# jxbi1010/VLA-Touch

Hardware: AMD Instinct MI355X
Metric: refined action chunks/sec (RDT-1B chunk + DINOv2 x2 + pi_I) (higher is better)
Workload: dtype bf16 model, 16-bit activations in IEEE fp16 (RDT-1B --rdt-compute f16, DINOv2 tower; same width and MFMA rate as bf16)

## Files before the change

### include/vlatouch.h

```cpp
#ifndef VLATOUCH_H
#define VLATOUCH_H
#include <stddef.h>
#include <stdint.h>
#ifdef __cplusplus
extern "C" {
#endif

typedef void* vt_stream_t;
typedef struct vt_unet_s* vt_unet_t;
typedef struct vt_dino_s* vt_dino_t;
typedef struct vt_lstm_s* vt_lstm_t;
typedef struct vt_rdt_s* vt_rdt_t;
typedef struct vt_t5_s* vt_t5_t;

const char* vt_last_error(void);
int vt_version(void);
int vt_selftest_mfma(float* out_err, vt_stream_t stream);

int vt_prof_enable(int on);
int vt_prof_collect(double* total_ms, double* flops, double* bytes, long* launches);

int vt_gemm(const void* params, vt_stream_t stream);
enum { VT_ROUTE_UNSUPPORTED = 0,
       VT_ROUTE_BAD_ARG = 1,
       VT_ROUTE_REG = 2,
       VT_ROUTE_F32R = 3,
       VT_ROUTE_GLDS = 4,
       VT_ROUTE_PP = 5,
       VT_ROUTE_PT = 6,
       VT_ROUTE_PPK = 7,
       VT_ROUTE_PW = 8,
       VT_ROUTE_PWS = 9,
       VT_ROUTE_ROWSPLIT = 10 };
int vt_gemm_route_of(const void* params);
int vt_gemm_route_split(const void* params, int* head_route, int* tail_route);
int vt_pack_w32(const void* W, long ldw, void* out, int N, int K, vt_stream_t stream);
int vt_tune(int knob, int value);

int vt_attention(const void* params, vt_stream_t stream);
int vt_attention_kvt(const void* params, vt_stream_t stream);
size_t vt_attention_kvt_part_bytes(int B, int H, int Nq, int parts);
int vt_retile_kv(const void* K, const void* V, long ld, void* KV, int M, int T, int H, vt_stream_t stream);
int vt_groupnorm(const void* params, vt_stream_t stream);
int vt_rownorm(const void* x, int xdt, long ldx, void* y, int ydt, long ldy, const float* w, const float* b,
               int rows, int D, float eps, int mode, vt_stream_t stream);
int vt_action_normalize(const float* in, float* out, const float* mins, const float* maxs, long n, int dim,
                        float padding_factor, int denormalize, vt_stream_t stream);
int vt_randn(float* out, long n, void* state, int round_bf16, vt_stream_t stream);
int vt_slice_cast(const void* in, int idt, float* out, int B, int Tin, int Din, int T, int Dd, vt_stream_t stream);
int vt_cast(const void* in, int idt, long ldi, void* out, int odt, long ldo, int rows, int cols, vt_stream_t stream);

typedef struct {
  int nets;
  int input_dim;
  int input_pad;
  int cond_dim;
  int dsed;
  int n_groups;
  int ksize;
  int n_levels;
  int dims[4];
  int cdt;
  int adt;
} vt_unet_desc;
int vt_unet_create(const vt_unet_desc* desc, const void* const* weights, int n_weights, vt_unet_t* out);
void vt_unet_destroy(vt_unet_t h);
int vt_unet_num_weights(const vt_unet_desc* desc);
size_t vt_unet_workspace_bytes(vt_unet_t h, int B, int T);
int vt_unet_forward(vt_unet_t h, const float* x, const float* t_dev, float t_host, const float* cond,
                    float* out, int B, int T, void* workspace, vt_stream_t stream);
int vt_si_sample(vt_unet_t h, float* x, const float* cond, const float* noise, int n_steps, float beta_max,
                 int gamma_type, int epsilon_type, int sde_type, float* traj, int B, int T, void* workspace,
                 vt_stream_t stream);
int vt_si_sample_ex(vt_unet_t h, float* x, const float* cond, const float* noise, int n_steps, float beta_max,
                    int gamma_type, int epsilon_type, int sde_type, int backward, float score_weight, float* traj,
                    int B, int T, void* workspace, vt_stream_t stream);
size_t vt_unet_fused_bytes(vt_unet_t h);
int vt_unet_fused_pack(vt_unet_t h, void* buf, vt_stream_t stream);
int vt_unet_fused_covers(vt_unet_t h, int B, int T, int n_steps);
size_t vt_unet_fused_plan_bytes(vt_unet_t h, int B, int T, int n_steps);
int vt_headnorm(void* x, int dt, long tok_stride, int heads, long tokens, const float* w, float eps, int mode,
                vt_stream_t stream);

typedef struct {
  int hidden, layers, heads, patch, kpad;
  int cdt, adt;
  float eps;
  int no_cls;
  int act;
  int head_dim;
  int mlp_dim;
  int out_all;
  float attn_scale;
} vt_dino_desc;
int vt_dino_create(const vt_dino_desc* desc, const void* const* weights, int n_weights, vt_dino_t* out);
void vt_dino_destroy(vt_dino_t h);
int vt_dino_num_weights(const vt_dino_desc* desc);
size_t vt_dino_workspace_bytes(vt_dino_t h, int B_total, int res);
size_t vt_dino_packed_bytes(vt_dino_t h);
int vt_dino_set_packed(vt_dino_t h, void* buf, vt_stream_t stream);
int vt_dino_set_range_flag(vt_dino_t h, unsigned* word);
int vt_dino_forward(vt_dino_t h, const void* const* imgs, int ncams, int is_u8, int nhwc, float pre_scale,
                    int norm_mode, int B, int res, const float* pos_patch, float* out, float* flags_out,
                    void* workspace, vt_stream_t stream);

typedef struct {
  int vocab, d_model, heads, d_kv, d_ff, layers;
  int num_buckets, max_distance;
  float eps;
  int cdt, adt;
} vt_t5_desc;
int vt_t5_create(const vt_t5_desc* desc, const void* const* weights, int n_weights, vt_t5_t* out);
void vt_t5_destroy(vt_t5_t h);
int vt_t5_num_weights(const vt_t5_desc* desc);
size_t vt_t5_workspace_bytes(vt_t5_t h, int B, int L);
int vt_t5_forward(vt_t5_t h, const int32_t* ids, const uint8_t* mask_or_null, int B, int L, const int8_t* bucket_tab, void* out, int out_dt,
                  void* workspace, vt_stream_t stream);

int vt_mlp(const void* x, long ldx, int B, int n_layers, const int* dims ,
           const void* const* W, const float* const* b, int act, void* y, int ydt, long ldy,
           int cdt, int adt, void* tmp, vt_stream_t stream);
int vt_concat_obs(const float* cls1, const float* cls2, int dv, const float* state, int sdim, const float* forces,
                  int fdim, void* out, int odt, long ldo, int B, vt_stream_t stream);

typedef struct { int state_dim, hidden, layers, force_dim, force_pad, in_pad, cdt; } vt_lstm_desc;
int vt_lstm_create(const vt_lstm_desc* desc, const void* const* weights, int n_weights, vt_lstm_t* out);
void vt_lstm_destroy(vt_lstm_t h);
int vt_lstm_num_weights(const vt_lstm_desc* desc);
size_t vt_lstm_workspace_bytes(vt_lstm_t h, int B);
int vt_lstm_step(vt_lstm_t hd, const float* obs_cond, const float* vla_n, const float* force, float* h, float* c,
                 float* out_n, int B, void* workspace, vt_stream_t stream);
int vt_lstm_sequence(vt_lstm_t hd, const float* obs_cond, const float* vla_n, const float* force, float* h, float* c,
                     float* out_n, int B, int T, vt_stream_t stream);

typedef struct {
  int hidden, depth, heads, horizon, out_dim;
  int state_dim;
  int lang_dim, img_dim;
  int max_lang_len, img_len;
  int n_lang, n_img, n_state;
  int cdt, adt;
  int rms_mode;
} vt_rdt_desc;
int vt_rdt_create(const vt_rdt_desc* desc, const void* const* weights, int n_weights, vt_rdt_t* out);
void vt_rdt_destroy(vt_rdt_t h);
int vt_rdt_num_weights(const vt_rdt_desc* desc);
size_t vt_rdt_workspace_bytes(vt_rdt_t h, int B, int lang_len);
int vt_rdt_set_score_bounds(vt_rdt_t h, const float* bounds, int n);
int vt_rdt_set_state_precision(vt_rdt_t h, int fp32_state);
int vt_rdt_set_io_dtype(vt_rdt_t h, int io_dtype);
size_t vt_rdt_packed_bytes(vt_rdt_t h);
int vt_rdt_set_packed(vt_rdt_t h, void* buf, vt_stream_t stream);
#ifndef VT_RANGE_XN_SAT
#define VT_RANGE_XN_SAT 1u
#define VT_RANGE_NONFINITE 2u
#define VT_RANGE_GATE_SAT 4u
#define VT_RANGE_ATTN_EMPTY 8u
#endif
int vt_rdt_set_range_flag(vt_rdt_t h, unsigned* word);
int vt_rdt_forward(vt_rdt_t h, const void* x_tokens, const float* freq, const float* t_dev, float t_host, int t_is_scalar,
                   const void* lang_c, const void* img_c, const uint8_t* lang_mask, void* out, int B, int L,
                   void* workspace, vt_stream_t stream);
int vt_rdt_sample(vt_rdt_t h, const void* lang_tokens, const uint8_t* lang_mask, const void* img_tokens,
                  const void* state_tokens, const void* action_mask, const float* ctrl_freqs, const float* x_init,
                  int n_steps, const float* timesteps, const float* coef, int sample_pred, int adapted, float* out,
                  int B, int L, void* workspace, vt_stream_t stream);

size_t vt_marker_workspace_bytes(int N, int H, int W, int max_cand);
int vt_marker_detect(const uint8_t* frames, int channels, int mode, int N, int H, int W, double min_area, double max_area,
                     int max_cand, int* markers, int* counts, int max_markers, uint8_t* binary_out, void* workspace,
                     vt_stream_t stream);
int vt_marker_displacement(const int* markers, const int* counts, int N, int max_markers, const int* baseline, int n_base,
                           int* disp, double* force, vt_stream_t stream);

int vt_im2col_t(const float* x, float* out, int B, int Tin, int Tout, int Cin, int taps, int stride, int off0, vt_stream_t stream);
int vt_transpose(const float* in, float* out, int M, int N, vt_stream_t stream);
int vt_zero_stuff(const float* x, float* out, int B, int T, int C, vt_stream_t stream);
int vt_wflip(const float* W, float* WT, int Cout, int taps, int Cin, vt_stream_t stream);
int vt_colsum(const float* x, long ld, float* out, int M, int N, int accumulate, vt_stream_t stream);
int vt_add_(float* a, const float* b, long n, vt_stream_t stream);
int vt_copy_cols(const float* src, long lds, int off, float* dst, long ldd, int doff, int rows, int cols, int accumulate, vt_stream_t stream);
int vt_mish(const float* x, const float* dy, float* out, long n, vt_stream_t stream);
int vt_gn_mish_bwd(const float* c, const float* gamma, const float* beta, const float* film, const float* dout, float* dc,
                   float* dgamma_part, float* dbeta_part, float* dfilm, int B, int T, int C, int ngroups, float eps, vt_stream_t stream);
int vt_gelu(const float* x, const float* dy, float* out, long n, vt_stream_t stream);
int vt_si_qsample(const float* x0, const float* x1, const float* z, const float* t, float* xt, float* target_v, float* target_s,
                  float* target_b, float* t_clipped, int B, long per_sample, int gamma_type, float t_min, vt_stream_t stream);
int vt_si_qsample_ex(const float* x0, const float* x1, const float* z, const float* t, float* xt, float* target_v, float* target_s,
                     float* target_b, float* t_clipped, int B, long per_sample, int gamma_type, float t_min, int interpolant_type, vt_stream_t stream);
int vt_si_loss(const float* out, const float* target, float* dout, float* loss, int B, long per_sample, vt_stream_t stream);
int vt_slab_sum(const float* slabs, int S, long n, const float* bias, int N, float* out, vt_stream_t stream);
int vt_adamw(float* p, const float* g, float* m, float* v, long n, float lr, float beta1, float beta2, float eps, float weight_decay,
             int step, vt_stream_t stream);
int vt_ema_update(float* shadow, const float* p, long n, float decay, vt_stream_t stream);
int vt_train_hyper(float lr, float beta1, float beta2, int step, float ema_decay, float* out4_host);
int vt_adamw_dev(float* p, const float* g, float* m, float* v, long n, const float* hyper, float beta1, float beta2, float eps,
                 float weight_decay, vt_stream_t stream);
int vt_adamw_ema_multi(const void* table, int ntensors, long total_chunks, const float* hyper, float beta1, float beta2, float eps,
                       float weight_decay, vt_stream_t stream);
int vt_ema_update_dev(float* shadow, const float* p, long n, const float* hyper, vt_stream_t stream);
int vt_posemb(const float* t, float* out, int B, int dim, vt_stream_t stream);

int vt_lstm_cell_fwd(const float* gx, const float* gh, float* act, float* cseq, float* hseq, float* hprev, float* hcur, int B, int T, int H,
                     int t, vt_stream_t stream);
int vt_lstm_cell_bwd(const float* dhseq, const float* dh_rec, const float* act, const float* cseq, float* dc_next, float* dgates, float* dgcur,
                     int B, int T, int H, int t, vt_stream_t stream);
int vt_ln_bwd(const float* x, const float* gamma, const float* dy, float* dx, float* dyxh, int rows, int C, float eps, vt_stream_t stream);
int vt_bcast_mid(const float* src, float* dst, long ldd, int doff, int B, int T, int C, vt_stream_t stream);
int vt_sum_mid(const float* src, long lds, int off, float* out, int B, int T, int C, vt_stream_t stream);
int vt_mul_(float* a, const float* b, long n, vt_stream_t stream);
int vt_mse_residual(const float* base, const float* delta, const float* target, float* pred, float* ddelta, float* loss, long n, vt_stream_t stream);

typedef struct {
  const void *Q, *K, *V, *dO;
  void *dQ, *dK, *dV;
  float* ws;
  const unsigned char* kmask;
  long km_bs;
  long q_bs, q_rs, q_hs, k_bs, k_rs, k_hs, v_bs, v_rs, v_hs, do_bs, do_rs, do_hs;
  long dq_bs, dq_rs, dq_hs, dk_bs, dk_rs, dk_hs, dv_bs, dv_rs, dv_hs;
  int B, H, Nq, Nk, hd, dtype;
  float scale;
} VtAttnBwdParams;
int vt_attention_bwd(const VtAttnBwdParams* params, vt_stream_t stream);
long vt_attention_bwd_mfma_ws_bytes(int B, int H, int Nq, int Nk);
int vt_attention_bwd_mfma(const VtAttnBwdParams* params, void* ws2, long ws2_bytes, vt_stream_t stream);
int vt_rmsnorm_bwd(const void* x, const float* w, const void* dy, void* dx, float* dyxr, int rows, int D, float eps, int mode, int dt, vt_stream_t stream);
int vt_headnorm_bwd(const void* x, long x_stride, void* dy, long dy_stride, int heads, long tokens, const float* w, float* part, float eps,
                    int mode, int dt, vt_stream_t stream);
int vt_act_bwd(const void* x, const void* dy, void* out, long n, int act, int dt, vt_stream_t stream);
int vt_ddpm_qsample(const float* state, const float* action, const float* noise, const float* mask, const long* timesteps,
                    const float* alphas_cumprod, int num_train_timesteps, void* out, int odt, int B, int horizon, int action_dim, vt_stream_t stream);
int vt_timestep_embed(const float* t, const float* freqs, void* out, int odt, int B, int dim, vt_stream_t stream);
int vt_add_rowvec_(void* a, int dt, const float* v, long rows, long cols, vt_stream_t stream);
int vt_transpose_pad(const void* in, void* out, int dt, int M, int N, int Mp, vt_stream_t stream);
int vt_colsum_dt(const void* x, int dt, long ld, float* out, int M, int N, vt_stream_t stream);
int vt_add_dt(void* a, const void* b, long n, int dt, vt_stream_t stream);
typedef struct {
  int splits, rows_per_split, m_step;
  long ws_bytes;
} VtGemmTnPlan;
int vt_gemm_tn_plan(int M, int N, int K, VtGemmTnPlan* plan);
int vt_gemm_tn(const void* dy, long ld_dy, const void* x, long ld_x, int dt, int M, int N, int K, float* dw, float* db, void* ws, long ws_bytes, vt_stream_t stream);
int vt_copy_cols_dt(const void* src, long lds, long off, void* dst, long ldd, long doff, long rows, long cols, int dt, vt_stream_t stream);
int vt_grad_clip_multi(const void* table, int ntensors, long total_chunks, float max_norm, float* chunk_part, float* norm_coef, vt_stream_t stream);
int vt_mse_loss(const void* pred, const float* target, void* dpred, float* loss, long n, int dt, vt_stream_t stream);
int vt_mse_loss_scaled(const void* pred, const float* target, void* dpred, float* loss, long n, int dt, float grad_scale, vt_stream_t stream);
int vt_grad_unscale_clip_multi(const void* table, int ntensors, long total_chunks, float max_norm, float inv_scale, float* chunk_part, float* norm_coef,
                               int* found_inf, vt_stream_t stream);
int vt_grad_accum_multi(const void* table, const void* fresh, int ntensors, long total_chunks, float scale, int accumulate, vt_stream_t stream);
int vt_ema_multi(const void* table, int ntensors, long total_chunks, const float* hyper, vt_stream_t stream);
int vt_grad_fold_pack_multi(const void* table, const void* fresh, int ntensors, long total_chunks, float scale, int accumulate, void* comm_bf16,
                            vt_stream_t stream);
int vt_grad_unpack_multi(const void* table, const void* comm_bf16, int ntensors, long total_chunks, vt_stream_t stream);
int vt_adamw8_ema_multi(const void* table, const void* aux, const float* tables, int ntensors, long total_chunks, const float* hyper, float beta1,
                        float beta2, float eps, float weight_decay, vt_stream_t stream);
int vt_adam8_quantize(const float* x, unsigned char* codes, float* absmax, const float* tables, int signed_table, long n, vt_stream_t stream);
int vt_adam8_dequantize(const unsigned char* codes, const float* absmax, const float* tables, int signed_table, float* out, long n, vt_stream_t stream);
int vt_sample_metrics(const void* pred, int dt, const float* target, const float* mask, const float* state_norm, const int* dataset_idx, int B,
                      int H, int A, int n_datasets, float* per_sample, float* overall, double* acc, int* count, double* ws, vt_stream_t stream);

typedef struct {
  const void* src;
  const void* coef_h;
  const void* coef_v;
  long pitch;
  int h, w;
  int out_h, out_w;
  int ksize_h, ksize_v;
  int rows_max;
  int reserved;
  long out_off;
  long ws_off;
} vt_imgprep_frame;
#define VT_IMGPREP_PAD 1
#define VT_IMGPREP_BRIGHT 2
#define VT_IMGPREP_OUT_BF16 4
#define VT_IMGPREP_OUT_U8 8
#define VT_IMGPREP_TWO_PASS 16
size_t vt_imgprep_workspace_bytes(vt_imgprep_frame* frames_host, int n, int S, int flags);
int vt_imgprep(const vt_imgprep_frame* frames_host, const void* frames_dev, int n, int S, const void* lut, unsigned fill_rgb, int flags,
               void* out, void* ws, size_t ws_bytes, vt_stream_t stream);

typedef struct {
  const void* src;
  long pitch;
  int h, w;
  long out_off;
  int order[4];
  float brightness, contrast, saturation;
  unsigned char hue_shift;
  unsigned char reserved[3];
} vt_colorjitter_frame;
#define VT_COLORJITTER_BRIGHTNESS 0
#define VT_COLORJITTER_CONTRAST 1
#define VT_COLORJITTER_SATURATION 2
#define VT_COLORJITTER_HUE 3
#define VT_COLORJITTER_NONE 4
#define VT_COLORJITTER_LIFT 1
size_t vt_colorjitter_workspace_bytes(int n);
int vt_colorjitter(const vt_colorjitter_frame* frames_host, const void* frames_dev, int n, int flags, void* out, void* ws, size_t ws_bytes,
                   vt_stream_t stream);

typedef struct {
  const void* src;
  long pitch;
  int h, w;
  long out_off;
  long ws_off;
} vt_jpegmap_frame;
#define VT_JPEGMAP_CV2_ORDER 1
size_t vt_jpegmap_workspace_bytes(vt_jpegmap_frame* frames_host, int n);
int vt_jpegmap(const vt_jpegmap_frame* frames_host, const void* frames_dev, int n, int quality, int flags, void* out, void* ws,
               size_t ws_bytes, vt_stream_t stream);

#define VT_RDT_MASK_FREQ 1
#define VT_RDT_MASK_STATE 2
#define VT_RDT_MASK_ELEM 4
#define VT_RDT_NOISE 8
int vt_rdt_batch(const double* qpos, const int* ep_off, const double* ep_stats, const double* ds_mean, const int* col_map, const float* lang,
                 const int* lang_off, int E, int S, int A, int H, int D, int Lmax, int ctrl_freq, double noise_div, const void* plan, int B,
                 float* states, float* actions, float* elem_mask, float* state_norm, long long* ctrl_freqs, float* lang_out,
                 unsigned char* lang_mask, vt_stream_t stream);

#define VT_CTRL_BRIDGE 0
#define VT_CTRL_LSTM 1
int vt_ctrl_batch(const double* pose10, const double* vla, const float* forces, const int* ep_off, const float* feat, const unsigned long long* pix_sum,
                  int E, long long rows, int Hv, int Fd, int dv, long long P, const float* stats, float padding_factor, int cf, int h, int layout,
                  int use_force, const int* plan, int B, float* obs_in, int in_pad, float* expert_act, float* vla_act, float* forces_out,
                  float* current_force, float* norm_flags, vt_stream_t stream);
int vt_ctrl_pixsum(const unsigned char* frames, long long P, int n, unsigned long long* sums, vt_stream_t stream);

#ifdef __cplusplus
}
#endif
#endif
```

### vla-touch_amd/csrc/vt_api.hip

```cpp
#include <string.h>
#include "vt_common.h"
#include "vt_kernels.h"
#include "vt_host.h"
#include "vt_gemm_route.h"
#include "vt_prof.h"
#include "vt_unet_int.h"
#include "../../include/vlatouch.h"

VtProfState g_vt_prof;

extern "C" {

const char* vt_last_error(void) { return vt_errbuf(); }
int vt_version(void) { return 100; }

int vt_gemm(const void* params, vt_stream_t stream) {
  if (!params) return vt_fail(VT_ERR_ARG, "vt_gemm: null params");
  const int r = vt_gemm_launch(*reinterpret_cast<const VtGemmParams*>(params), (hipStream_t)stream);
  if (r) vt_fail(r, "vt_gemm: rejected (alignment: K, lda, ldw multiples of 8 bf16 / 4 fp32; conv: cin likewise) or launch failure");
  return r;
}
int vt_gemm_route_of(const void* params) {
  if (!params) return VT_ROUTE_BAD_ARG;
  return vt_gemm_route(*reinterpret_cast<const VtGemmParams*>(params));
}
int vt_gemm_route_split(const void* params, int* head_route, int* tail_route) {
  if (!params || !head_route || !tail_route) return vt_fail(VT_ERR_ARG, "vt_gemm_route_split: null argument");
  const VtGemmParams& p = *reinterpret_cast<const VtGemmParams*>(params);
  if (vt_gemm_route(p) != VT_GEMM_ROWSPLIT) return vt_fail(VT_ERR_ARG, "vt_gemm_route_split: the block does not route to VT_ROUTE_ROWSPLIT");
  VtGemmParams head, tail;
  *head_route = vt_gemm_rowsplit(p, head, tail);
  *tail_route = vt_gemm_route(tail);
  return VT_OK;
}
int vt_tune(int knob, int value) {
  if (knob == 1 && (value == 0 || value == 4 || value == 8)) { vt_gemm_pw_tune(value); return VT_OK; }
  if (knob == 2 || knob == 8) { vt_gemm_route_tune(knob, value); return VT_OK; }
  if (knob == 4) { vt_gemm_pws_tune(value); return VT_OK; }
  if (knob == 6) { vt_attn_kvt_tune(value); return VT_OK; }
  if (knob == 7) { vt_unet_fused_tune(value); return VT_OK; }
  if (knob == 9 && (value == 0 || value == 1 || value == 3 || value == 6)) { vt_attn16g_tune(value); return VT_OK; }
  return vt_fail(VT_ERR_ARG, "vt_tune: unknown knob %d / value %d", knob, value);
}
int vt_prof_enable(int on) {
  g_vt_prof.on = on != 0;
  g_vt_prof.mode = on > 1 ? on : 1;
  if (on) { g_vt_prof.used = 0; g_vt_prof.flops = 0.0; g_vt_prof.bytes = 0.0; }
  return VT_OK;
}
int vt_prof_collect(double* total_ms, double* flops, double* bytes, long* launches) {
  double ms = 0.0;
  for (int i = 0; i < g_vt_prof.used; ++i) {
    float t = 0.f;
    if (hipEventElapsedTime(&t, g_vt_prof.ev[2 * i], g_vt_prof.ev[2 * i + 1]) != hipSuccess) return VT_ERR_LAUNCH;
    ms += t;
  }
  if (total_ms) *total_ms = ms;
  if (flops) *flops = g_vt_prof.flops;
  if (bytes) *bytes = g_vt_prof.bytes;
  if (launches) *launches = g_vt_prof.used;
  return VT_OK;
}
int vt_attention(const void* params, vt_stream_t stream) {
  if (!params) return vt_fail(VT_ERR_ARG, "vt_attention: null params");
  const int r = vt_attn_launch(*reinterpret_cast<const VtAttnParams*>(params), (hipStream_t)stream);
  if (r) vt_fail(r, "vt_attention: bad strides/sizes or launch failure");
  return r;
}
int vt_attention_kvt(const void* params, vt_stream_t stream) {
  if (!params) return vt_fail(VT_ERR_ARG, "vt_attention_kvt: null params");
  const int r = vt_attn_kvt_launch(*reinterpret_cast<const VtAttnKvtParams*>(params), (hipStream_t)stream);
  if (r) vt_fail(r, "vt_attention_kvt: bad sizes / strides (T * 64 >= B * Nk, q_rs % 8), parts without part_ws or > 16, or launch failure");
  return r;
}
size_t vt_attention_kvt_part_bytes(int B, int H, int Nq, int parts) { return vt_attn_kvt_part_bytes(B, H, Nq, parts); }
int vt_retile_kv(const void* K, const void* V, long ld, void* KV, int M, int T, int H, vt_stream_t stream) {
  if (!K || !V || !KV || M < 1 || H < 1) return vt_fail(VT_ERR_ARG, "vt_retile_kv: null source / destination or empty shape");
  const int r = vt_k_retile_kv(K, V, ld, KV, M, T, H, (hipStream_t)stream);
  if (r) vt_fail(r, "vt_retile_kv: T * 64 < M, ld % 8 or launch failure");
  return r;
}
int vt_groupnorm(const void* params, vt_stream_t stream) {
  if (!params) return vt_fail(VT_ERR_ARG, "vt_groupnorm: null params");
  const int r = vt_k_groupnorm(*reinterpret_cast<const VtGnParams*>(params), (hipStream_t)stream);
  if (r) vt_fail(r, "vt_groupnorm: unsupported group size or launch failure");
  return r;
}
int vt_rownorm(const void* x, int xdt, long ldx, void* y, int ydt, long ldy, const float* w, const float* b, int rows, int D, float eps,
               int mode, vt_stream_t stream) {
  const int r = vt_k_rownorm(x, xdt, ldx, y, ydt, ldy, w, b, rows, D, eps, mode, (hipStream_t)stream);
  if (r) vt_fail(r, "vt_rownorm: D must be a multiple of 4 and <= 2048");
  return r;
}
int vt_headnorm(void* x, int dt, long tok_stride, int heads, long tokens, const float* w, float eps, int mode, vt_stream_t stream) {
  return vt_k_headnorm(x, dt, tok_stride, heads, tokens, w, eps, mode, (hipStream_t)stream);
}
int vt_action_normalize(const float* in, float* out, const float* mins, const float* maxs, long n, int dim, float padding_factor,
                        int denormalize, vt_stream_t stream) {
  if (!in || !out || !mins || !maxs || n < 0 || dim < 1) return vt_fail(VT_ERR_ARG, "vt_action_normalize: bad argument");
  if (n == 0) return VT_OK;
  return vt_k_actnorm(in, out, mins, maxs, n, dim, padding_factor, denormalize, (hipStream_t)stream);
}

}

static_assert(VT_ROUTE_UNSUPPORTED == VT_GEMM_UNSUPPORTED && VT_ROUTE_BAD_ARG == VT_GEMM_BAD_ARG && VT_ROUTE_REG == VT_GEMM_REG && VT_ROUTE_F32R == VT_GEMM_F32R &&
              VT_ROUTE_GLDS == VT_GEMM_GLDS && VT_ROUTE_PP == VT_GEMM_PP && VT_ROUTE_PT == VT_GEMM_PT && VT_ROUTE_PPK == VT_GEMM_PPK && VT_ROUTE_PW == VT_GEMM_PW &&
              VT_ROUTE_PWS == VT_GEMM_PWS && VT_ROUTE_ROWSPLIT == VT_GEMM_ROWSPLIT, "include/vlatouch.h route codes = enum VtGemmRoute");

namespace {
template <typename T>
__global__ void mfma_selftest_kernel(float* err) {
  const int lane = threadIdx.x, g = lane >> 4, l15 = lane & 15;
  Frag<T> a, b;
  float av[8], bv[8];
  for (int j = 0; j < 8; ++j) {
    const int k = g * 8 + j;
    av[j] = (k == l15) ? 1.f : 0.f;
    bv[j] = (float)(l15 * 100 + k);
  }
  if constexpr (sizeof(T) == 2) {
    for (int j = 0; j < 8; ++j) { a.v[j] = (short)f2bf(av[j]); b.v[j] = (short)f2bf(bv[j]); }
  } else {
    for (int j = 0; j < 8; ++j) { a.v[j] = av[j]; b.v[j] = bv[j]; }
  }
  float4_t acc = {0.f, 0.f, 0.f, 0.f};
  mma16(acc, a, b);
  float e = 0.f;
  for (int r = 0; r < 4; ++r) {
    const int row = g * 4 + r, col = l15;
    float expect = (float)(col * 100 + row);
    if constexpr (sizeof(T) == 2) expect = bf2f(f2bf(expect));
    e = fmaxf(e, fabsf(acc[r] - expect));
  }
  e = wave_max(e);
  if (lane == 0) *err = e;
}
}

extern "C" int vt_selftest_mfma(float* out_err, vt_stream_t stream) {
  if (!out_err) return vt_fail(VT_ERR_ARG, "vt_selftest_mfma: null");
  hipLaunchKernelGGL((mfma_selftest_kernel<bf16_t>), dim3(1), dim3(64), 0, (hipStream_t)stream, out_err);
  hipLaunchKernelGGL((mfma_selftest_kernel<float>), dim3(1), dim3(64), 0, (hipStream_t)stream, out_err + 1);
  return vt_check_launch();
}

namespace {
__device__ __forceinline__ void philox_round(uint32_t (&c)[4], const uint32_t k0, const uint32_t k1) {
  const uint64_t p0 = (uint64_t)0xD2511F53u * c[0], p1 = (uint64_t)0xCD9E8D57u * c[2];
  const uint32_t n0 = (uint32_t)(p1 >> 32) ^ c[1] ^ k0, n1 = (uint32_t)p1, n2 = (uint32_t)(p0 >> 32) ^ c[3] ^ k1, n3 = (uint32_t)p0;
  c[0] = n0; c[1] = n1; c[2] = n2; c[3] = n3;
}
__device__ __forceinline__ void philox4x32_10(uint32_t (&c)[4], uint32_t k0, uint32_t k1) {
#pragma unroll
  for (int r = 0; r < 10; ++r) { philox_round(c, k0, k1); k0 += 0x9E3779B9u; k1 += 0xBB67AE85u; }
}
__global__ void randn_kernel(float* __restrict__ out, const long n, const unsigned long long* __restrict__ state, const int round_bf16) {
  const long q = (long)blockIdx.x * blockDim.x + threadIdx.x;
  if (q * 4 >= n) return;
  const unsigned long long key = state[0], ctr = state[1] + (unsigned long long)q;
  uint32_t c[4] = {(uint32_t)ctr, (uint32_t)(ctr >> 32), 0u, 0u};
  philox4x32_10(c, (uint32_t)key, (uint32_t)(key >> 32));
  float v[4];
#pragma unroll
  for (int h = 0; h < 2; ++h) {
    const float u1 = ((float)(c[2 * h] >> 8) + 0.5f) * (1.0f / 16777216.0f);
    const float u2 = ((float)(c[2 * h + 1] >> 8) + 0.5f) * (1.0f / 16777216.0f);
    const float r = sqrtf(-2.0f * __logf(u1));
    float sn, cs;
    __sincosf(6.283185307179586f * u2, &sn, &cs);
    v[2 * h] = r * cs; v[2 * h + 1] = r * sn;
  }
#pragma unroll
  for (int j = 0; j < 4; ++j) {
    if (round_bf16) v[j] = bf2f(f2bf(v[j]));
    if (q * 4 + j < n) out[q * 4 + j] = v[j];
  }
}
__global__ void randn_advance_kernel(unsigned long long* state, const unsigned long long by) { state[1] += by; }
template <typename TI>
__global__ void slice_cast_kernel(const TI* __restrict__ in, float* __restrict__ out, int B, int Tin, int Din, int T, int Dd) {
  const long i = (long)blockIdx.x * blockDim.x + threadIdx.x;
  if (i >= (long)B * T * Dd) return;
  const int d = (int)(i % Dd);
  const long r = i / Dd;
  const int t = (int)(r % T), b = (int)(r / T);
  out[i] = Elem<TI>::to_f(in[((long)b * Tin + t) * Din + d]);
}
}

extern "C" int vt_randn(float* out, long n, void* state, int round_bf16, vt_stream_t stream) {
  if (!out || !state || n < 0) return vt_fail(VT_ERR_ARG, "vt_randn: null argument");
  if (n == 0) return VT_OK;
  const long quads = (n + 3) / 4;
  hipLaunchKernelGGL(randn_kernel, dim3((unsigned)((quads + 255) / 256)), dim3(256), 0, (hipStream_t)stream, out, n, (const unsigned long long*)state, round_bf16);
  hipLaunchKernelGGL(randn_advance_kernel, dim3(1), dim3(1), 0, (hipStream_t)stream, (unsigned long long*)state, (unsigned long long)quads);
  return vt_check_launch();
}
extern "C" int vt_slice_cast(const void* in, int idt, float* out, int B, int Tin, int Din, int T, int Dd, vt_stream_t stream) {
  if (!in || !out || B < 1 || T < 1 || Dd < 1 || T > Tin || Dd > Din) return vt_fail(VT_ERR_ARG, "vt_slice_cast: bad shape");
  const long n = (long)B * T * Dd;
  const dim3 grid((unsigned)((n + 255) / 256));
  if (idt == VT_BF16) hipLaunchKernelGGL((slice_cast_kernel<bf16_t>), grid, dim3(256), 0, (hipStream_t)stream, (const bf16_t*)in, out, B, Tin, Din, T, Dd);
  else if (idt == VT_F32) hipLaunchKernelGGL((slice_cast_kernel<float>), grid, dim3(256), 0, (hipStream_t)stream, (const float*)in, out, B, Tin, Din, T, Dd);
  else return vt_fail(VT_ERR_UNSUPPORTED, "vt_slice_cast: bf16 or fp32 input");
  return vt_check_launch();
}

extern "C" int vt_cast(const void* in, int idt, long ldi, void* out, int odt, long ldo, int rows, int cols, vt_stream_t stream) {
  if (!in || !out || rows < 1 || cols < 1) return vt_fail(VT_ERR_ARG, "vt_cast: bad argument");
  const int r = vt_k_act_copy(in, idt, ldi, out, odt, ldo, rows, cols, VT_ACT_NONE, (hipStream_t)stream);
  if (r) vt_fail(r, "vt_cast: unsupported dtype pair");
  return r;
}
```

### vla-touch_amd/csrc/vt_common.h

```cpp
#pragma once
#include <hip/hip_runtime.h>
#include <stdint.h>
#include <type_traits>

typedef uint16_t bf16_t;
typedef __attribute__((ext_vector_type(8))) short short8_t;
typedef __attribute__((ext_vector_type(4))) float float4_t;
typedef __attribute__((ext_vector_type(8))) __bf16 bf16x8_t;
typedef __attribute__((ext_vector_type(8))) _Float16 f16x8_t;
struct half_t { uint16_t b; };
typedef __attribute__((ext_vector_type(4))) short short4_t;
typedef __attribute__((ext_vector_type(4))) int int4_t;
typedef __attribute__((ext_vector_type(16))) float float16_t;
typedef __attribute__((address_space(3))) void lds_void;
typedef const __attribute__((address_space(1))) void glb_void;
typedef __attribute__((address_space(3))) short4_t lds_short4_t;

#define VT_OK 0
#define VT_ERR_ARG (-22)
#define VT_ERR_LAUNCH (-5)
#define VT_ERR_UNSUPPORTED (-95)

enum { VT_F32 = 0, VT_BF16 = 1, VT_F32X3 = 2, VT_F16 = 3 };
enum { VT_ACT_NONE = 0, VT_ACT_GELU_ERF = 1, VT_ACT_GELU_TANH = 2, VT_ACT_SILU = 3, VT_ACT_MISH = 4,
       VT_ACT_SWIGLU = 5,
       VT_ACT_GEGLU = 6 };

__device__ __forceinline__ float bf2f(bf16_t h) { return __uint_as_float(((uint32_t)h) << 16); }
typedef __attribute__((ext_vector_type(2))) float float2_t;
typedef __attribute__((ext_vector_type(2))) __bf16 bf16x2_t;
__device__ __forceinline__ uint32_t pk_bf16(float lo, float hi) {
  return __builtin_bit_cast(uint32_t, __builtin_convertvector((float2_t){lo, hi}, bf16x2_t));
}
typedef __attribute__((ext_vector_type(2))) _Float16 f16x2_t;
template <typename T> __device__ __forceinline__ uint32_t pk16(float lo, float hi);
template <> __device__ __forceinline__ uint32_t pk16<bf16_t>(float lo, float hi) { return pk_bf16(lo, hi); }
template <> __device__ __forceinline__ uint32_t pk16<half_t>(float lo, float hi) {
  return __builtin_bit_cast(uint32_t, __builtin_convertvector((float2_t){lo, hi}, f16x2_t));
}
template <typename T> __host__ __device__ constexpr short one16() { return std::is_same<T, half_t>::value ? (short)0x3C00 : (short)0x3F80; }
__device__ __forceinline__ bf16_t f2bf(float f) { return __builtin_bit_cast(bf16_t, (__bf16)f); }
__device__ __forceinline__ float h2f(half_t h) { return (float)__builtin_bit_cast(_Float16, h.b); }
__device__ __forceinline__ half_t f2h(float f) { half_t r; r.b = __builtin_bit_cast(uint16_t, (_Float16)f); return r; }

template <typename T> struct Elem;
template <> struct Elem<float> {
  static constexpr int EPC = 4;
  __device__ static __forceinline__ float to_f(float v) { return v; }
  __device__ static __forceinline__ float from_f(float v) { return v; }
};
template <> struct Elem<bf16_t> {
  static constexpr int EPC = 8;
  __device__ static __forceinline__ float to_f(bf16_t v) { return bf2f(v); }
  __device__ static __forceinline__ bf16_t from_f(float v) { return f2bf(v); }
};
template <> struct Elem<half_t> {
  static constexpr int EPC = 8;
  __device__ static __forceinline__ float to_f(half_t v) { return h2f(v); }
  __device__ static __forceinline__ half_t from_f(float v) { return f2h(v); }
};

template <typename T> struct Frag;
template <> struct Frag<bf16_t> { short8_t v; };
template <> struct Frag<half_t> { short8_t v; };
template <> struct Frag<float> { float v[8]; };

__device__ __forceinline__ void mma16(float4_t& acc, const Frag<bf16_t>& a, const Frag<bf16_t>& b) {
  acc = __builtin_amdgcn_mfma_f32_16x16x32_bf16(__builtin_bit_cast(bf16x8_t, a.v), __builtin_bit_cast(bf16x8_t, b.v), acc, 0, 0, 0);
}
__device__ __forceinline__ void mma16(float4_t& acc, const Frag<half_t>& a, const Frag<half_t>& b) {
  acc = __builtin_amdgcn_mfma_f32_16x16x32_f16(__builtin_bit_cast(f16x8_t, a.v), __builtin_bit_cast(f16x8_t, b.v), acc, 0, 0, 0);
}
__device__ __forceinline__ void mma16(float4_t& acc, const Frag<float>& a, const Frag<float>& b) {
#pragma unroll
  for (int j = 0; j < 8; ++j) acc = __builtin_amdgcn_mfma_f32_16x16x4f32(a.v[j], b.v[j], acc, 0, 0, 0);
}

template <typename T16> __device__ __forceinline__ float16_t mma32(const int4_t w, const int4_t a, const float16_t c);
template <> __device__ __forceinline__ float16_t mma32<bf16_t>(const int4_t w, const int4_t a, const float16_t c) {
  return __builtin_amdgcn_mfma_f32_32x32x16_bf16(__builtin_bit_cast(bf16x8_t, w), __builtin_bit_cast(bf16x8_t, a), c, 0, 0, 0);
}
template <> __device__ __forceinline__ float16_t mma32<half_t>(const int4_t w, const int4_t a, const float16_t c) {
  return __builtin_amdgcn_mfma_f32_32x32x16_f16(__builtin_bit_cast(f16x8_t, w), __builtin_bit_cast(f16x8_t, a), c, 0, 0, 0);
}

template <int N, typename F> __device__ __forceinline__ void static_for(F&& f) {
  if constexpr (N > 0) { static_for<N - 1>(f); f(std::integral_constant<int, N - 1>{}); }
}

#ifdef VLATOUCH_DRAIN_WAITS
#define VT_VMCNT(N) 0
#else
#define VT_VMCNT(N) N
#endif
template <int N> __device__ __forceinline__ void vt_wait_vm() { asm volatile("s_waitcnt vmcnt(%0)" ::"n"(VT_VMCNT(N)) : "memory"); }
template <int N> __device__ __forceinline__ void vt_wait_vm(int4_t (&w)[4]) {
  asm volatile("s_waitcnt vmcnt(%[n])" : "+v"(w[0]), "+v"(w[1]), "+v"(w[2]), "+v"(w[3]) : [n] "i"(VT_VMCNT(N)) : "memory");
}
template <int N> __device__ __forceinline__ void vt_wait_vm(int4_t (&w)[8]) {
  asm volatile("s_waitcnt vmcnt(%[n])" : "+v"(w[0]), "+v"(w[1]), "+v"(w[2]), "+v"(w[3]), "+v"(w[4]), "+v"(w[5]), "+v"(w[6]), "+v"(w[7]) : [n] "i"(VT_VMCNT(N)) : "memory");
}

template <int OFF, bool FIRST>
__device__ __forceinline__ void wload(int4_t& d, const unsigned voff, const char* sbase) {
  if constexpr (FIRST) asm volatile("s_nop 4\n\tglobal_load_dwordx4 %0, %1, %2 offset:%3" : "=v"(d) : "v"(voff), "s"(sbase), "i"(OFF) : "memory");
  else asm volatile("global_load_dwordx4 %0, %1, %2 offset:%3" : "=v"(d) : "v"(voff), "s"(sbase), "i"(OFF) : "memory");
}
#define VT_UNIFORM_PTR(p)                                                                                                             \
  reinterpret_cast<const char*>(((unsigned long)(unsigned)__builtin_amdgcn_readfirstlane((int)((unsigned long)(p) >> 32)) << 32) | \
                                (unsigned long)(unsigned)__builtin_amdgcn_readfirstlane((int)(unsigned long)(p)))

__device__ __forceinline__ int swz(int row, int chunk) { return chunk ^ ((row >> 1) & 7); }

__device__ __forceinline__ void lds_frag(Frag<bf16_t>& f, const char* tile, int row, int k8) {
  f.v = *reinterpret_cast<const short8_t*>(tile + row * 128 + swz(row, k8) * 16);
}
__device__ __forceinline__ void lds_frag(Frag<half_t>& f, const char* tile, int row, int k8) {
  f.v = *reinterpret_cast<const short8_t*>(tile + row * 128 + swz(row, k8) * 16);
}
__device__ __forceinline__ void lds_frag(Frag<float>& f, const char* tile, int row, int k8) {
  const float4_t lo = *reinterpret_cast<const float4_t*>(tile + row * 128 + swz(row, 2 * k8) * 16);
  const float4_t hi = *reinterpret_cast<const float4_t*>(tile + row * 128 + swz(row, 2 * k8 + 1) * 16);
  f.v[0] = lo[0]; f.v[1] = lo[1]; f.v[2] = lo[2]; f.v[3] = lo[3];
  f.v[4] = hi[0]; f.v[5] = hi[1]; f.v[6] = hi[2]; f.v[7] = hi[3];
}

template <typename T>
__device__ __forceinline__ void tr_frag_half(Frag<T>& f, const int hh, const char* a) {
  const short4_t t = __builtin_amdgcn_ds_read_tr16_b64_v4i16((lds_short4_t*)a);
  f.v[hh * 4 + 0] = t[0]; f.v[hh * 4 + 1] = t[1]; f.v[hh * 4 + 2] = t[2]; f.v[hh * 4 + 3] = t[3];
}

__device__ __forceinline__ float fast_exp(float x) { return __builtin_amdgcn_exp2f(x * 1.4426950408889634f); }

__device__ __forceinline__ float fast_erf(float x) {
  const float ax = fabsf(x);
  const float t = __builtin_amdgcn_rcpf(1.0f + 0.3275911f * ax);
  const float p = t * (0.254829592f + t * (-0.284496736f + t * (1.421413741f + t * (-1.453152027f + t * 1.061405429f))));
  return copysignf(1.0f - p * fast_exp(-ax * ax), x);
}

__device__ __forceinline__ float act_apply(float x, int act) {
  switch (act) {
    case VT_ACT_GELU_ERF: return 0.5f * x * (1.0f + fast_erf(x * 0.70710678118654752440f));
    case VT_ACT_GELU_TANH: {
      const float u2 = 1.5957691216057308f * (x + 0.044715f * x * x * x);
      return x * __builtin_amdgcn_rcpf(1.0f + fast_exp(-u2));
    }
    case VT_ACT_SILU: return x * __builtin_amdgcn_rcpf(1.0f + fast_exp(-x));
    case VT_ACT_MISH: {
      if (x > 20.0f) return x;
      const float n = fast_exp(x), w = n * (n + 2.0f);
      return x * w * __builtin_amdgcn_rcpf(w + 2.0f);
    }
    default: return x;
  }
}

template <int W, bool MAX> __device__ __forceinline__ float rows_pair(float v) {
  static_assert(W == 16 || W == 32, "a row is 16 lanes: pairs of rows, then pairs of pairs");
  const unsigned u = __builtin_bit_cast(unsigned, v);
  float a0, a1;
  if constexpr (W == 16) {
    const auto a = __builtin_amdgcn_permlane16_swap(u, u, false, false);
    a0 = __builtin_bit_cast(float, (unsigned)a[0]); a1 = __builtin_bit_cast(float, (unsigned)a[1]);
  } else {
    const auto a = __builtin_amdgcn_permlane32_swap(u, u, false, false);
    a0 = __builtin_bit_cast(float, (unsigned)a[0]); a1 = __builtin_bit_cast(float, (unsigned)a[1]);
  }
  return MAX ? fmaxf(a0, a1) : a0 + a1;
}
__device__ __forceinline__ float rows4_sum(float v) { return rows_pair<32, false>(rows_pair<16, false>(v)); }
__device__ __forceinline__ float rows4_max(float v) { return rows_pair<32, true>(rows_pair<16, true>(v)); }
__device__ __forceinline__ float row16_sum(float v) {
  auto dpp = [](float x, auto ctrl) {
    return __int_as_float(__builtin_amdgcn_update_dpp(0, __float_as_int(x), decltype(ctrl)::value, 0xf, 0xf, false));
  };
  v += dpp(v, std::integral_constant<int, 0xB1>{});
  v += dpp(v, std::integral_constant<int, 0x4E>{});
  v += dpp(v, std::integral_constant<int, 0x141>{});
  v += dpp(v, std::integral_constant<int, 0x140>{});
  return v;
}
__device__ __forceinline__ float row16_max(float v) {
  auto dpp = [](float x, auto ctrl) {
    return __int_as_float(__builtin_amdgcn_update_dpp(0, __float_as_int(x), decltype(ctrl)::value, 0xf, 0xf, false));
  };
  v = fmaxf(v, dpp(v, std::integral_constant<int, 0xB1>{}));
  v = fmaxf(v, dpp(v, std::integral_constant<int, 0x4E>{}));
  v = fmaxf(v, dpp(v, std::integral_constant<int, 0x141>{}));
  v = fmaxf(v, dpp(v, std::integral_constant<int, 0x140>{}));
  return v;
}
__device__ __forceinline__ float wave_sum(float v) { return rows4_sum(row16_sum(v)); }
__device__ __forceinline__ float wave_max(float v) { return rows4_max(row16_max(v)); }

template <typename T> __device__ __forceinline__ float ldf(const T* p, size_t i);
template <> __device__ __forceinline__ float ldf<float>(const float* p, size_t i) { return p[i]; }
template <> __device__ __forceinline__ float ldf<bf16_t>(const bf16_t* p, size_t i) { return bf2f(p[i]); }
template <> __device__ __forceinline__ float ldf<half_t>(const half_t* p, size_t i) { return h2f(p[i]); }
template <typename T> __device__ __forceinline__ void stf(T* p, size_t i, float v);
template <> __device__ __forceinline__ void stf<float>(float* p, size_t i, float v) { p[i] = v; }
template <> __device__ __forceinline__ void stf<bf16_t>(bf16_t* p, size_t i, float v) { p[i] = f2bf(v); }
template <> __device__ __forceinline__ void stf<half_t>(half_t* p, size_t i, float v) { p[i] = f2h(v); }

__device__ __forceinline__ float vt_actnorm(float x, float mn, float mx, float pad, int denorm) {
  const float pr = (mx - mn) * pad;
  const float ctr = (mn + mx) / 2;
  const float pmin = ctr - pr / 2, pmax = ctr + pr / 2;
  float rng = pmax - pmin;
  if (denorm) return (x + 1.0f) / 2.0f * rng + pmin;
  if (rng < 1e-6f) rng = 1.0f;
  return 2.0f * (x - pmin) / rng - 1.0f;
}

#ifndef VT_RANGE_XN_SAT
#define VT_RANGE_XN_SAT 1u
#define VT_RANGE_NONFINITE 2u
#define VT_RANGE_GATE_SAT 4u
#define VT_RANGE_ATTN_EMPTY 8u
#endif
__device__ __forceinline__ void vt_range_note(unsigned* flag, unsigned bit) {
  if (flag) __hip_atomic_fetch_or(flag, bit, __ATOMIC_RELAXED, __HIP_MEMORY_SCOPE_AGENT);
}
__device__ __forceinline__ bool vt_nonfinite(float v) { return !(fabsf(v) <= 3.4028234664e38f); }

static inline int vt_check_launch() { return hipGetLastError() == hipSuccess ? VT_OK : VT_ERR_LAUNCH; }

#define DISPATCH_T(dt, T, ...) \
  if ((dt) == VT_F32) { using T = float; __VA_ARGS__; } else if ((dt) == VT_F16) { using T = half_t; __VA_ARGS__; } else { using T = bf16_t; __VA_ARGS__; }
#define DISPATCH_T16(dt, T, ...) \
  if ((dt) == VT_F16) { using T = half_t; __VA_ARGS__; } else { using T = bf16_t; __VA_ARGS__; }
static inline bool vt_is_act_dtype(int dt) { return dt == VT_F32 || dt == VT_BF16 || dt == VT_F16; }
```

### vla-touch_amd/csrc/vt_gemm_pw.hip

```cpp
#include "vt_common.h"
#include "vt_gemm_route.h"
#include "vt_gemm_epilogue.h"
#include "vt_prof.h"
#include "vt_host.h"
#include "vt_kernels.h"
#include "../../include/vlatouch.h"

namespace {

constexpr int BM = 160, BN = 128, BK = 64;
constexpr int TMW = BM / 32;
constexpr int A_TILE = BM * 128;
constexpr int OPS = BM / 8 / 4 + 4;

template <typename T16, typename TC, int NB, int FUSE = 0>
__global__ __launch_bounds__(256, 1) void gemm_pw_kernel(const VtGemmParams p, const int tiles_n, const int tiles_per_group, const int total_tiles, const int GM) {
  constexpr int SMEM = NB * A_TILE > BM * BN * 4 ? NB * A_TILE : BM * BN * 4;
  __shared__ __attribute__((aligned(16))) char smem[SMEM];
  const int tid = threadIdx.x, lane = tid & 63;
  const int wave = __builtin_amdgcn_readfirstlane(tid >> 6);
  const int l31 = lane & 31, hk = lane >> 5;

  int bid = blockIdx.x;
  if ((total_tiles & 7) == 0) bid = (bid & 7) * (total_tiles >> 3) + (bid >> 3);
  const int grp = bid / tiles_per_group;
  const int t_in = bid - grp * tiles_per_group;
  const int tiles_m = tiles_per_group / tiles_n;
  const int sr = t_in / (GM * tiles_n);
  const int gmr = min(GM, tiles_m - sr * GM);
  const int r_in = t_in - sr * GM * tiles_n;
  const int tn = r_in / gmr, tm = sr * GM + (r_in - tn * gmr);
  const int m0 = tm * BM, n0 = tn * BN;

  const uint16_t* A = reinterpret_cast<const uint16_t*>(p.A) + (long)grp * p.a_gs;
  const int nk = p.K / BK;

  const __amdgpu_buffer_rsrc_t rsA = __builtin_amdgcn_make_buffer_rsrc((void*)(A + (long)m0 * p.lda), 0, 0x7fffffff, 0x00020000);
  int asrc[5];
#pragma unroll
  for (int e = 0; e < 5; ++e) {
    const int r = (wave + 4 * e) * 8 + (lane >> 3);
    const int c = (lane & 7) ^ ((r >> 1) & 7);
    asrc[e] = (int)(((long)(min(m0 + r, p.M - 1) - m0) * p.lda + c * 8) * 2);
  }
  const char* wbase = reinterpret_cast<const char*>(p.Wp) + ((long)grp * p.w_gs) * 2 + ((long)(n0 / 32 + wave) * (p.K / 16)) * 1024;
  wbase = VT_UNIFORM_PTR(wbase);
  const unsigned wvoff = lane * 16;

  int4_t wb[NB][4];
  auto issue = [&](const int kt, auto bc) {
    constexpr int b = decltype(bc)::value;
#pragma unroll
    for (int e = 0; e < 5; ++e)
      __builtin_amdgcn_raw_ptr_buffer_load_lds(rsA, (lds_void*)(smem + b * A_TILE + (wave + 4 * e) * 1024), 16, asrc[e], kt * (BK * 2), 0, 0);
    const char* sb = wbase + (long)kt * 4096;
    wload<0, true>(wb[b][0], wvoff, sb);
    wload<1024, false>(wb[b][1], wvoff, sb);
    wload<2048, false>(wb[b][2], wvoff, sb);
    wload<3072, false>(wb[b][3], wvoff, sb);
  };

  const int xr = (l31 >> 1) & 7;
  int foff[4];
#pragma unroll
  for (int s = 0; s < 4; ++s) foff[s] = l31 * 128 + (((s * 2 + hk) ^ xr) * 16);
  auto frags = [&](int4_t (&f)[TMW], const int b, const int s) {
#pragma unroll
    for (int j = 0; j < TMW; ++j) f[j] = *reinterpret_cast<const int4_t*>(smem + b * A_TILE + j * 4096 + foff[s]);
  };

  float16_t acc[TMW];
#pragma unroll
  for (int j = 0; j < TMW; ++j)
#pragma unroll
    for (int r = 0; r < 16; ++r) acc[j][r] = 0.f;

  static_for<NB - 1>([&](auto bc) { if (decltype(bc)::value < nk) issue(decltype(bc)::value, bc); });
  vt_wait_vm<(NB - 3) * OPS>(wb[0]);
  vt_wait_vm<(NB - 3) * OPS>(wb[1]);
  __builtin_amdgcn_sched_barrier(0);
  __builtin_amdgcn_s_barrier();
  __builtin_amdgcn_sched_barrier(0);
  int4_t af[2][TMW];
  frags(af[0], 0, 0);

  constexpr int RSV = FUSE == 2 ? (BM * 16 + 255) / 256 : 1;
  float4 rsv[RSV];
  auto sub = [&](const int t, auto uc, auto tailc) {
    constexpr int U = decltype(uc)::value;
    constexpr bool TAIL = decltype(tailc)::value;
    if constexpr (!TAIL || U == 0) issue(t + NB - 1, std::integral_constant<int, (U + NB - 1) % NB>{});
    if constexpr (FUSE == 2 && TAIL && U == NB - 2) {
      const int h2 = p.rs_n >> 1, nq = BM * h2;
#pragma unroll
      for (int i = 0; i < RSV; ++i) {
        const int q = tid + 256 * i;
        const int row = q / h2, c = q - row * h2;
        rsv[i] = q < nq ? *reinterpret_cast<const float4*>(p.rs_part + ((long)min(m0 + row, p.M - 1) * p.rs_n + 2 * c) * 2) : make_float4(0.f, 0.f, 0.f, 0.f);
      }
    }
#pragma unroll
    for (int s = 0; s < 4; ++s) {
      if (s < 3) frags(af[(s + 1) & 1], U, s + 1);
      else if (!TAIL || U < NB - 1) frags(af[0], (U + 1) % NB, 0);
#pragma unroll
      for (int j = 0; j < TMW; ++j) acc[j] = mma32<T16>(wb[U][s], af[s & 1][j], acc[j]);
    }
#pragma unroll
    for (int i = 0; i < 4 * TMW; ++i) {
      __builtin_amdgcn_sched_group_barrier(0x008, 1, 0);
      __builtin_amdgcn_sched_group_barrier(0x100, 1, 0);
    }
    if constexpr (!TAIL) vt_wait_vm<(NB - 3) * OPS>(wb[(U + 2) % NB]);
    else if constexpr (U + 2 < NB) vt_wait_vm<(NB - 3 - U > 0 ? NB - 3 - U : 0) * OPS>(wb[(U + 2) % NB]);
    __builtin_amdgcn_sched_barrier(0);
    __builtin_amdgcn_s_barrier();
    __builtin_amdgcn_sched_barrier(0);
  };
  int t = 0;
  for (; t + NB < nk; t += NB) static_for<NB>([&](auto uc) { sub(t + decltype(uc)::value, uc, std::false_type{}); });
  static_for<NB>([&](auto uc) { sub(t + decltype(uc)::value, uc, std::true_type{}); });

  float* tile = reinterpret_cast<float*>(smem);
  float rs[TMW];
#pragma unroll
  for (int j = 0; j < TMW; ++j) rs[j] = 1.f;
  if constexpr (FUSE == 2) {
    float2* pair = reinterpret_cast<float2*>(tile + BM);
    const int h2 = p.rs_n >> 1;
#pragma unroll
    for (int i = 0; i < RSV; ++i) {
      const int q = tid + 256 * i;
      if (q < BM * h2) {
        const float dS = rsv[i].y - rsv[i].w;
        pair[q] = make_float2(rsv[i].x + rsv[i].z + (p.rs_mode == 2 ? dS * dS * (1.0f / 128.0f) : 0.f), rsv[i].y + rsv[i].w);
      }
    }
    __syncthreads();
    if (tid < BM) {
      float var;
      if (p.rs_mode == 2) {
        float na = 0.f, mean = 0.f, m2 = 0.f;
        for (int c = 0; c < h2; ++c) {
          const float2 v = pair[tid * h2 + c];
          const float delta = v.y * (1.0f / 128.0f) - mean, nt = na + 128.0f;
          mean += delta * (128.0f / nt);
          m2 += v.x + delta * delta * (na * 128.0f / nt);
          na = nt;
        }
        var = m2 / (1.0f / p.rs_inv_k - 1.0f);
      } else {
        float sq = 0.f;
        for (int c = 0; c < h2; ++c) sq += pair[tid * h2 + c].x;
        var = sq * p.rs_inv_k;
      }
      tile[tid] = rsqrtf(var + p.rs_eps);
    }
    __syncthreads();
#pragma unroll
    for (int j = 0; j < TMW; ++j) rs[j] = tile[j * 32 + l31];
    __syncthreads();
  }
  const int half = wave & 1, c4 = lane & 15;
  const int ncol0 = n0 + half * 64, n = ncol0 + c4 * 4;
  const bool col_ok = n < p.N;
  const int rbase = (wave >> 1) * (BM / 2) + (lane >> 4);
  TC* Cg = reinterpret_cast<TC*>(p.C) + (long)grp * p.c_gs;
  const TC* Rg = p.residual ? reinterpret_cast<const TC*>(p.residual) + (long)grp * p.r_gs : nullptr;
  constexpr bool PRE = sizeof(TC) == 4;
  float4 rpre[PRE ? BM / 8 : 1];
  const bool use_pre = PRE && Rg != nullptr;
  if constexpr (PRE) {
    if (use_pre) {
#pragma unroll
      for (int it = 0; it < BM / 8; ++it) {
        const int m = min(m0 + rbase + it * 4, p.M - 1);
        rpre[it] = col_ok ? *reinterpret_cast<const float4*>(reinterpret_cast<const float*>(Rg) + (long)m * p.ldr + n) : make_float4(0.f, 0.f, 0.f, 0.f);
      }
    }
  }
  const float* bias = p.bias ? p.bias + (long)grp * p.bias_gs : nullptr;
  const float* hw = nullptr;
  if (p.hn_w0 && ncol0 < p.hn_c0_end) hw = p.hn_w0;
  else if (p.hn_w1 && ncol0 >= p.hn_c0_end && ncol0 < p.hn_c1_end) hw = p.hn_w1;
  const float4 zero4 = make_float4(0.f, 0.f, 0.f, 0.f), one4 = make_float4(1.f, 1.f, 1.f, 1.f);
  const float4 b4 = (bias && col_ok) ? *reinterpret_cast<const float4*>(bias + n) : zero4;
  const float4 cs4 = (p.colscale && col_ok) ? *reinterpret_cast<const float4*>(p.colscale + n) : one4;
  const float4 hw4 = hw ? *reinterpret_cast<const float4*>(hw + c4 * 4) : one4;
  float4 g4 = zero4;
  if constexpr (FUSE == 1) { if (col_ok && p.xn_gain) g4 = *reinterpret_cast<const float4*>(p.xn_gain + n); }
  __builtin_amdgcn_sched_barrier(0);
  constexpr int PFN = 8;
  unsigned pfv[PFN];
#pragma unroll
  for (int i = 0; i < PFN; ++i) pfv[i] = 0;
  if (p.pf_ptr) {
    const unsigned nbytes = (unsigned)p.pf_bytes;
    const unsigned share = ((nbytes + (unsigned)total_tiles - 1u) / (unsigned)total_tiles + 63u) & ~63u;
    const unsigned b0 = blockIdx.x * share;
    const __amdgpu_buffer_rsrc_t rsP = __builtin_amdgcn_make_buffer_rsrc((void*)((const char*)p.pf_ptr + b0), 0,
                                                                        b0 < nbytes ? (int)min(share, nbytes - b0) : 0, 0x00020000);
#pragma unroll
    for (int i = 0; i < PFN; ++i)
      if ((unsigned)i * 16384u < share) pfv[i] = __builtin_amdgcn_raw_buffer_load_b32(rsP, (i * 256 + tid) * 64, 0, 0);
  }
  __builtin_amdgcn_sched_barrier(0);
#pragma unroll
  for (int j = 0; j < TMW; ++j) {
    const int m = j * 32 + l31;
    const float r = FUSE == 2 ? rs[j] : 1.f;
#pragma unroll
    for (int rq = 0; rq < 4; ++rq) {
      const int n4 = wave * 8 + rq * 2 + hk;
      *reinterpret_cast<float4*>(tile + m * BN + ((n4 ^ (m & 7)) * 4)) =
          make_float4(acc[j][rq * 4] * r, acc[j][rq * 4 + 1] * r, acc[j][rq * 4 + 2] * r, acc[j][rq * 4 + 3] * r);
    }
  }
  __syncthreads();
  if (p.act != VT_ACT_NONE) {
#pragma unroll 2
    for (int it = 0; it < BM / 8; ++it) {
      const int row = rbase + it * 4;
      const float4 x = *reinterpret_cast<const float4*>(tile + row * BN + (((half * 16 + c4) ^ (row & 7)) * 4));
      vt_epi_segment<TC, 0, true>(p, x, b4, cs4, hw, hw4, Cg, Rg, m0 + row, n, ncol0, col_ok);
    }
  } else if (FUSE == 1 && PRE && use_pre) {
    if constexpr (PRE && FUSE == 1) {
      T16* Xn = reinterpret_cast<T16*>(p.xn_out);
      const int pcol = 2 * tn + half, pn = 2 * tiles_n;
#pragma unroll
      for (int it = 0; it < BM / 8; ++it) {
        const int row = rbase + it * 4, m = m0 + row;
        const float4 x = *reinterpret_cast<const float4*>(tile + row * BN + (((half * 16 + c4) ^ (row & 7)) * 4));
        float o[4] = {x.x + b4.x, x.y + b4.y, x.z + b4.z, x.w + b4.w};
        o[0] *= cs4.x; o[1] *= cs4.y; o[2] *= cs4.z; o[3] *= cs4.w;
        o[0] += rpre[it].x; o[1] += rpre[it].y; o[2] += rpre[it].z; o[3] += rpre[it].w;
        const bool ok = m < p.M && col_ok;
        const float q1 = row16_sum(ok ? (o[0] + o[1]) + (o[2] + o[3]) : 0.f);
        float q;
        if (p.rs_mode == 2) {
          const float mj = q1 * (1.0f / 64.0f);
          const float d0 = o[0] - mj, d1 = o[1] - mj, d2 = o[2] - mj, d3 = o[3] - mj;
          q = row16_sum(ok ? (d0 * d0 + d1 * d1) + (d2 * d2 + d3 * d3) : 0.f);
        } else q = row16_sum(ok ? (o[0] * o[0] + o[1] * o[1]) + (o[2] * o[2] + o[3] * o[3]) : 0.f);
        if (ok) {
          vt_epi_st128(reinterpret_cast<float*>(Cg) + (long)m * p.ldc + n, make_float4(o[0], o[1], o[2], o[3]));
          constexpr float LIM = std::is_same<T16, half_t>::value ? 65504.0f : 3.0e38f;
          auto sat = [](float v) { return fminf(fmaxf(v, -LIM), LIM); };
          const float xg[4] = {o[0] * g4.x, o[1] * g4.y, o[2] * g4.z, o[3] * g4.w};
          if constexpr (std::is_same<T16, half_t>::value) {
            if (fmaxf(fmaxf(fabsf(xg[0]), fabsf(xg[1])), fmaxf(fabsf(xg[2]), fabsf(xg[3]))) > LIM) vt_range_note(p.range_flag, VT_RANGE_XN_SAT);
          }
          T16 ov[4] = {Elem<T16>::from_f(sat(xg[0])), Elem<T16>::from_f(sat(xg[1])), Elem<T16>::from_f(sat(xg[2])), Elem<T16>::from_f(sat(xg[3]))};
          vt_epi_st64(Xn + (long)m * p.xn_ld + n, *reinterpret_cast<const uint2*>(ov));
        }
        if (c4 == 0 && m < p.M) *reinterpret_cast<float2*>(p.xn_part + ((long)m * pn + pcol) * 2) = make_float2(q, q1);
      }
    }
  } else if (use_pre) {
#pragma unroll
    for (int it = 0; it < BM / 8; ++it) {
      const int row = rbase + it * 4;
      const float4 x = *reinterpret_cast<const float4*>(tile + row * BN + (((half * 16 + c4) ^ (row & 7)) * 4));
      vt_epi_segment<TC, 0, false>(p, x, b4, cs4, hw, hw4, Cg, nullptr, m0 + row, n, ncol0, col_ok, &rpre[PRE ? it : 0]);
    }
  } else {
#pragma unroll 4
    for (int it = 0; it < BM / 8; ++it) {
      const int row = rbase + it * 4;
      const float4 x = *reinterpret_cast<const float4*>(tile + row * BN + (((half * 16 + c4) ^ (row & 7)) * 4));
      vt_epi_segment<TC, 0, false>(p, x, b4, cs4, hw, hw4, Cg, Rg, m0 + row, n, ncol0, col_ok);
    }
  }
#pragma unroll
  for (int i = 0; i < PFN; ++i) asm volatile("" :: "v"(pfv[i]));
}

__global__ void pack_w32_kernel(const uint16_t* __restrict__ W, const long ldw, uint16_t* __restrict__ out, const int N, const int K) {
  const long i = (long)blockIdx.x * blockDim.x + threadIdx.x;
  const long nchunks = (long)N * K / 8;
  if (i >= nchunks) return;
  const int lane = (int)(i & 63);
  const long frag = i >> 6;
  const int ks = (int)(frag % (K / 16));
  const int nt = (int)(frag / (K / 16));
  const int n = nt * 32 + (lane & 31), k = ks * 16 + (lane >> 5) * 8;
  *reinterpret_cast<uint4*>(out + i * 8) = *reinterpret_cast<const uint4*>(W + (long)n * ldw + k);
}

}

static int g_vt_pw_nb = 0;

void vt_gemm_pw_tune(int ring) { g_vt_pw_nb = ring; }

bool vt_gemm_pw_fits(const VtGemmParams& p) {
  if (!p.Wp || p.cmap || p.groups != 1) return false;
  if (p.N % BN || p.K % (8 * BK) || p.lda >= (1 << 21)) return false;
  const long tiles = (long)((p.M + BM - 1) / BM) * (p.N / BN) * p.groups;
  const long rounds = (tiles + 255) / 256;
  return tiles >= 100 && tiles * 8 >= rounds * 256 * 7;
}

int vt_gemm_pw_launch(const VtGemmParams& p, hipStream_t s) {
  const int tiles_n = p.N / BN, tiles_m = (p.M + BM - 1) / BM;
  const int per_group = tiles_n * tiles_m, total = per_group * p.groups;
  const int gm = 4;
  VtProfScope prof(3, p, s);
  const bool c16 = p.c_dtype != VT_F32;
#define VT_PW_GO(T16, TC) do { if (g_vt_pw_nb == 8) hipLaunchKernelGGL((gemm_pw_kernel<T16, TC, 8>), dim3(total), dim3(256), 0, s, p, tiles_n, per_group, total, gm); \
                               else hipLaunchKernelGGL((gemm_pw_kernel<T16, TC, 4>), dim3(total), dim3(256), 0, s, p, tiles_n, per_group, total, gm); } while (0)
  if (p.xn_out || p.rs_part) {
    const dim3 g(total), b(256);
    if (p.xn_out && (c16 || !p.residual || p.act != VT_ACT_NONE || p.hn_w0 || p.hn_w1)) return VT_ERR_UNSUPPORTED;
    if (p.xn_out && p.rs_part) return VT_ERR_UNSUPPORTED;
    if (p.xn_out) {
      if (p.a_dtype == VT_BF16) hipLaunchKernelGGL((gemm_pw_kernel<bf16_t, float, 4, 1>), g, b, 0, s, p, tiles_n, per_group, total, gm);
      else hipLaunchKernelGGL((gemm_pw_kernel<half_t, float, 4, 1>), g, b, 0, s, p, tiles_n, per_group, total, gm);
    } else if (!c16) {
      return VT_ERR_UNSUPPORTED;
    } else if (p.a_dtype == VT_BF16) {
      hipLaunchKernelGGL((gemm_pw_kernel<bf16_t, bf16_t, 4, 2>), g, b, 0, s, p, tiles_n, per_group, total, gm);
    } else {
      hipLaunchKernelGGL((gemm_pw_kernel<half_t, half_t, 4, 2>), g, b, 0, s, p, tiles_n, per_group, total, gm);
    }
    return vt_check_launch();
  }
  if (p.a_dtype == VT_BF16) { if (c16) VT_PW_GO(bf16_t, bf16_t); else VT_PW_GO(bf16_t, float); }
  else { if (c16) VT_PW_GO(half_t, half_t); else VT_PW_GO(half_t, float); }
#undef VT_PW_GO
  return vt_check_launch();
}

extern "C" int vt_pack_w32(const void* W, long ldw, void* out, int N, int K, vt_stream_t stream) {
  if (!W || !out || N <= 0 || K <= 0 || N % 32 || K % 16 || ldw % 8) return vt_fail(VT_ERR_ARG, "vt_pack_w32: N %% 32, K %% 16, ldw %% 8 must be 0");
  const long nchunks = (long)N * K / 8;
  hipLaunchKernelGGL(pack_w32_kernel, dim3((unsigned)((nchunks + 255) / 256)), dim3(256), 0, (hipStream_t)stream, (const uint16_t*)W, ldw, (uint16_t*)out, N, K);
  return vt_check_launch();
}
```

### vla-touch_amd/csrc/vt_gemm_route.h

```cpp
#pragma once
#include <hip/hip_runtime.h>
#include "vt_gemm.h"

enum VtGemmRoute : int {
  VT_GEMM_UNSUPPORTED = 0,
  VT_GEMM_BAD_ARG = 1,
  VT_GEMM_REG = 2,
  VT_GEMM_F32R = 3,
  VT_GEMM_GLDS = 4,
  VT_GEMM_PP = 5,
  VT_GEMM_PT = 6,
  VT_GEMM_PPK = 7,
  VT_GEMM_PW = 8,
  VT_GEMM_PWS = 9,
  VT_GEMM_ROWSPLIT = 10,
};

VtGemmRoute vt_gemm_route(const VtGemmParams& p);
VtGemmRoute vt_gemm_rowsplit(const VtGemmParams& p, VtGemmParams& head, VtGemmParams& tail);
void vt_gemm_route_tune(int knob, int value);

bool vt_gemm_lds_fits(const VtGemmParams& p);
bool vt_gemm_can_fuse_headnorm(const VtGemmParams& p);
bool vt_gemm_pp_fits(const VtGemmParams& p);
bool vt_gemm_pt_fits(const VtGemmParams& p);
bool vt_gemm_pt_one_round(const VtGemmParams& p);
bool vt_gemm_ppk_fits(const VtGemmParams& p);
bool vt_gemm_pw_fits(const VtGemmParams& p);
bool vt_gemm_pws_fits(const VtGemmParams& p);
bool vt_gemm_f32r_fits(const VtGemmParams& p);

int vt_gemm_reg_launch(const VtGemmParams& p, hipStream_t s);
int vt_gemm_f32r_launch(const VtGemmParams& p, hipStream_t s);
int vt_gemm_fast_launch(const VtGemmParams& p, hipStream_t s);
int vt_gemm_pp_launch(const VtGemmParams& p, hipStream_t s);
int vt_gemm_pt_launch(const VtGemmParams& p, hipStream_t s);
int vt_gemm_ppk_launch(const VtGemmParams& p, hipStream_t s);
int vt_gemm_pw_launch(const VtGemmParams& p, hipStream_t s);
int vt_gemm_pws_launch(const VtGemmParams& p, hipStream_t s);
void vt_gemm_pw_tune(int ring);
void vt_gemm_pws_tune(int split);
```

### vla-touch_amd/csrc/vt_gemm_route.hip

```cpp
#include "vt_common.h"
#include "vt_gemm_route.h"
#include "vt_kernels.h"

static int g_pw_on = 1;
static int g_pt_on = 1;

void vt_gemm_route_tune(int knob, int value) { (knob == 2 ? g_pw_on : g_pt_on) = value != 0; }

static bool sq256(const VtGemmParams& p) { return vt_gemm_pp_fits(p) || (g_pt_on && vt_gemm_pt_one_round(p)); }
static VtGemmRoute sq256_route(const VtGemmParams& p) { return g_pt_on && vt_gemm_pt_fits(p) ? VT_GEMM_PT : VT_GEMM_PP; }

static int rowsplit_rows(const VtGemmParams& p) {
  if (p.cmap != 0 || p.groups != 1 || p.hn_w0 || p.hn_w1 || p.M % 256 == 0 || p.M % 256 > 64 || !sq256(p)) return 0;
  const long tm = (p.M + 255) / 256, tn = (p.N + 255) / 256;
  if (tm <= 1 || (tm * tn + 255) / 256 <= ((tm - 1) * tn + 255) / 256) return 0;
  VtGemmParams a = p;
  a.M = (int)((tm - 1) * 256);
  return vt_gemm_lds_fits(a) && sq256(a) ? a.M : 0;
}

VtGemmRoute vt_gemm_rowsplit(const VtGemmParams& p, VtGemmParams& head, VtGemmParams& tail) {
  head = p; tail = p;
  head.M = rowsplit_rows(p);
  const size_t ea = p.a_dtype == VT_F32 ? 4 : 2, ec = p.c_dtype == VT_F32 ? 4 : 2;
  tail.M = p.M - head.M;
  tail.A = (const char*)p.A + (size_t)head.M * p.lda * ea;
  tail.C = (char*)p.C + (size_t)head.M * p.ldc * ec;
  if (p.residual) tail.residual = (const char*)p.residual + (size_t)head.M * p.ldr * ec;
  return sq256_route(head);
}

VtGemmRoute vt_gemm_route(const VtGemmParams& p) {
  if (p.M <= 0 || p.N <= 0 || p.K <= 0) return VT_GEMM_BAD_ARG;
  const int epc = p.w_dtype == VT_F32 ? 4 : 8;
  if (p.K % epc || p.ldw % epc || p.lda % epc) return VT_GEMM_BAD_ARG;
  if (p.taps && (p.cin % epc || p.K != p.taps * p.cin)) return VT_GEMM_BAD_ARG;
  if (p.splitk < 1 || p.groups < 1) return VT_GEMM_BAD_ARG;
  if (p.splitk > 1 && p.c_dtype != VT_F32) return VT_GEMM_BAD_ARG;
  if (p.pf_ptr && p.pf_bytes >= (1ul << 31)) return VT_GEMM_BAD_ARG;
  const bool hn = p.hn_w0 || p.hn_w1;
  const bool lds = vt_gemm_lds_fits(p);
  const bool pw = lds && g_pw_on && vt_gemm_pw_fits(p);
  if (p.xn_out || p.rs_part) {
    if (p.groups != 1 || (p.xn_out && (!p.xn_gain || !p.xn_part || p.c_dtype != VT_F32 || !p.residual || p.act != VT_ACT_NONE || hn || p.xn_ld % 4)) ||
        (p.rs_part && (p.rs_n < 4 || p.rs_n > 32 || p.rs_n % 4)) || !pw)
      return VT_GEMM_UNSUPPORTED;
    return VT_GEMM_PW;
  }
  if (vt_gemm_pws_fits(p) && (p.M <= 192 || !lds)) return VT_GEMM_PWS;
  if (lds) {
    if (pw) return VT_GEMM_PW;
    if (rowsplit_rows(p)) return VT_GEMM_ROWSPLIT;
    if (sq256(p)) return sq256_route(p);
    if (vt_gemm_ppk_fits(p)) return VT_GEMM_PPK;
    return VT_GEMM_GLDS;
  }
  if (hn || p.cmap) return VT_GEMM_UNSUPPORTED;
  const int a = p.a_dtype, w = p.w_dtype, c = p.c_dtype;
  if (a == VT_BF16 && w == VT_BF16) return c == VT_BF16 || c == VT_F32 ? VT_GEMM_REG : VT_GEMM_UNSUPPORTED;
  if (a == VT_F16 && w == VT_F16) return c == VT_F16 || c == VT_F32 ? VT_GEMM_REG : VT_GEMM_UNSUPPORTED;
  if (a == VT_F32 && w == VT_BF16) return VT_GEMM_REG;
  if (vt_gemm_f32r_fits(p)) return VT_GEMM_F32R;
  if (a == VT_F32 && (w == VT_F32 || w == VT_F32X3) && c == VT_F32) return VT_GEMM_REG;
  return VT_GEMM_UNSUPPORTED;
}

int vt_gemm_launch(const VtGemmParams& p, hipStream_t s) {
  switch (vt_gemm_route(p)) {
    case VT_GEMM_BAD_ARG: return VT_ERR_ARG;
    case VT_GEMM_UNSUPPORTED: return VT_ERR_UNSUPPORTED;
    case VT_GEMM_REG: return vt_gemm_reg_launch(p, s);
    case VT_GEMM_F32R: return vt_gemm_f32r_launch(p, s);
    case VT_GEMM_GLDS: return vt_gemm_fast_launch(p, s);
    case VT_GEMM_PP: return vt_gemm_pp_launch(p, s);
    case VT_GEMM_PT: return vt_gemm_pt_launch(p, s);
    case VT_GEMM_PPK: return vt_gemm_ppk_launch(p, s);
    case VT_GEMM_PW: return vt_gemm_pw_launch(p, s);
    case VT_GEMM_PWS: return vt_gemm_pws_launch(p, s);
    case VT_GEMM_ROWSPLIT: {
      VtGemmParams head, tail;
      const int rc = vt_gemm_rowsplit(p, head, tail) == VT_GEMM_PT ? vt_gemm_pt_launch(head, s) : vt_gemm_pp_launch(head, s);
      return rc != VT_OK ? rc : vt_gemm_launch(tail, s);
    }
  }
  return VT_ERR_UNSUPPORTED;
}
```

### vla-touch_amd/vlatouch/_lib.py

```python
from __future__ import annotations

import ctypes as C
import os
from typing import Optional, Sequence

import torch

_HERE = os.path.dirname(os.path.abspath(__file__))
LIB_PATH = os.environ.get("VLATOUCH_LIB") or os.path.join(_HERE, "libvlatouch_hip.so")

RANGE_XN_SAT, RANGE_NONFINITE, RANGE_GATE_SAT, RANGE_ATTN_EMPTY = 1, 2, 4, 8
RANGE_NAMES = {RANGE_XN_SAT: "xn_saturated", RANGE_NONFINITE: "nonfinite", RANGE_GATE_SAT: "gate_saturated", RANGE_ATTN_EMPTY: "attention_row_empty"}


def csrc_sha16() -> str:
    import glob
    import hashlib
    h = hashlib.sha256()
    d = os.path.join(os.path.dirname(_HERE), "csrc")
    for f in sorted(glob.glob(os.path.join(d, "*.hip")) + glob.glob(os.path.join(d, "*.h")) + [os.path.join(d, "Makefile")]):
        h.update(os.path.basename(f).encode())
        h.update(open(f, "rb").read())
    return h.hexdigest()[:16]


def range_names(bits: int):
    return [n for b, n in RANGE_NAMES.items() if bits & b]


F32, BF16, F32X3, F16 = 0, 1, 2, 3
ACT_NONE, ACT_GELU_ERF, ACT_GELU_TANH, ACT_SILU, ACT_MISH, ACT_SWIGLU, ACT_GEGLU = 0, 1, 2, 3, 4, 5, 6
ROUTE_NAMES = ("UNSUPPORTED", "BAD_ARG", "REG", "F32R", "GLDS", "PP", "PT", "PPK", "PW", "PWS", "ROWSPLIT")
NORM_LAYER, NORM_RMS_MEANSQ, NORM_RMS_VAR = 0, 1, 2
IMGNORM_AUTO, IMGNORM_ON, IMGNORM_OFF = 0, 1, 2


class VtError(RuntimeError):
    pass


class GemmParams(C.Structure):
    _fields_ = [
        ("A", C.c_void_p), ("W", C.c_void_p), ("C", C.c_void_p),
        ("M", C.c_int), ("N", C.c_int), ("K", C.c_int),
        ("lda", C.c_long), ("ldw", C.c_long), ("ldc", C.c_long),
        ("taps", C.c_int), ("cin", C.c_int), ("tout", C.c_int), ("tin", C.c_int), ("stride", C.c_int),
        ("off0", C.c_int), ("tstep", C.c_int),
        ("bias", C.c_void_p), ("colscale", C.c_void_p), ("residual", C.c_void_p), ("ldr", C.c_long),
        ("act", C.c_int),
        ("groups", C.c_int), ("splitk", C.c_int),
        ("a_gs", C.c_long), ("w_gs", C.c_long), ("c_gs", C.c_long), ("bias_gs", C.c_long), ("r_gs", C.c_long),
        ("c_slab", C.c_long),
        ("a_dtype", C.c_int), ("w_dtype", C.c_int), ("c_dtype", C.c_int),
        ("hn_w0", C.c_void_p), ("hn_w1", C.c_void_p), ("hn_c0_end", C.c_int), ("hn_c1_end", C.c_int),
        ("hn_eps", C.c_float), ("hn_mode", C.c_int),
        ("cmap", C.c_int), ("cmap_T", C.c_int),
        ("Wp", C.c_void_p),
        ("sk_ws", C.c_void_p), ("sk_ws_bytes", C.c_size_t), ("sk_cnt", C.c_void_p), ("sk_cnt_n", C.c_int),
        ("xn_out", C.c_void_p), ("xn_ld", C.c_long), ("xn_gain", C.c_void_p), ("xn_part", C.c_void_p),
        ("rs_part", C.c_void_p), ("rs_n", C.c_int), ("rs_inv_k", C.c_float), ("rs_eps", C.c_float), ("rs_mode", C.c_int),
        ("pf_ptr", C.c_void_p), ("pf_bytes", C.c_size_t),
        ("range_flag", C.c_void_p),
    ]


class GnParams(C.Structure):
    _fields_ = [
        ("P", C.c_void_p), ("nslabs", C.c_int), ("slab_stride", C.c_long), ("p_gs", C.c_long), ("ldp", C.c_long),
        ("bias", C.c_void_p), ("gamma", C.c_void_p), ("beta", C.c_void_p), ("vec_gs", C.c_long),
        ("film", C.c_void_p), ("film_ld", C.c_long), ("film_off", C.c_long), ("film_gs", C.c_long),
        ("residual", C.c_void_p), ("ldr", C.c_long), ("r_gs", C.c_long),
        ("out", C.c_void_p), ("ldo", C.c_long), ("o_gs", C.c_long), ("out_dtype", C.c_int),
        ("B", C.c_int), ("T", C.c_int), ("C", C.c_int), ("ngroups", C.c_int), ("nets", C.c_int),
        ("eps", C.c_float),
    ]


class AttnParams(C.Structure):
    _fields_ = [
        ("Q", C.c_void_p), ("K", C.c_void_p), ("V", C.c_void_p), ("O", C.c_void_p),
        ("q_bs", C.c_long), ("q_rs", C.c_long), ("q_hs", C.c_long),
        ("k_bs", C.c_long), ("k_rs", C.c_long), ("k_hs", C.c_long),
        ("v_bs", C.c_long), ("v_rs", C.c_long), ("v_hs", C.c_long),
        ("o_bs", C.c_long), ("o_rs", C.c_long),
        ("kmask", C.c_void_p), ("km_bs", C.c_long),
        ("B", C.c_int), ("H", C.c_int), ("Nq", C.c_int), ("Nk", C.c_int),
        ("scale", C.c_float), ("dtype", C.c_int), ("hd", C.c_int),
    ]


class AttnKvtParams(C.Structure):
    _fields_ = [
        ("Q", C.c_void_p), ("KV", C.c_void_p), ("O", C.c_void_p),
        ("q_bs", C.c_long), ("q_rs", C.c_long),
        ("o_bs", C.c_long), ("o_rs", C.c_long),
        ("kmask", C.c_void_p),
        ("B", C.c_int), ("H", C.c_int), ("Nq", C.c_int), ("Nk", C.c_int), ("T", C.c_int),
        ("scale", C.c_float),
        ("parts", C.c_int),
        ("part_ws", C.c_void_p),
        ("fixed_max", C.c_float),
        ("dtype", C.c_int),
        ("range_flag", C.c_void_p),
    ]


class AttnBwdParams(C.Structure):
    _fields_ = ([(n, C.c_void_p) for n in ("Q", "K", "V", "dO", "dQ", "dK", "dV", "ws", "kmask")] + [("km_bs", C.c_long)] +
                [(f"{t}_{s}", C.c_long) for t in ("q", "k", "v", "do", "dq", "dk", "dv") for s in ("bs", "rs", "hs")] +
                [(n, C.c_int) for n in ("B", "H", "Nq", "Nk", "hd", "dtype")] + [("scale", C.c_float)])


class GemmTnPlan(C.Structure):
    _fields_ = [("splits", C.c_int), ("rows_per_split", C.c_int), ("m_step", C.c_int), ("ws_bytes", C.c_long)]


class UnetDesc(C.Structure):
    _fields_ = [("nets", C.c_int), ("input_dim", C.c_int), ("input_pad", C.c_int), ("cond_dim", C.c_int),
                ("dsed", C.c_int), ("n_groups", C.c_int), ("ksize", C.c_int), ("n_levels", C.c_int),
                ("dims", C.c_int * 4), ("cdt", C.c_int), ("adt", C.c_int)]


class DinoDesc(C.Structure):
    _fields_ = [("hidden", C.c_int), ("layers", C.c_int), ("heads", C.c_int), ("patch", C.c_int), ("kpad", C.c_int),
                ("cdt", C.c_int), ("adt", C.c_int), ("eps", C.c_float),
                ("no_cls", C.c_int), ("act", C.c_int), ("head_dim", C.c_int), ("mlp_dim", C.c_int), ("out_all", C.c_int),
                ("attn_scale", C.c_float)]


class T5Desc(C.Structure):
    _fields_ = [("vocab", C.c_int), ("d_model", C.c_int), ("heads", C.c_int), ("d_kv", C.c_int), ("d_ff", C.c_int), ("layers", C.c_int),
                ("num_buckets", C.c_int), ("max_distance", C.c_int), ("eps", C.c_float), ("cdt", C.c_int), ("adt", C.c_int)]


class ImgprepFrame(C.Structure):
    _fields_ = [("src", C.c_void_p), ("coef_h", C.c_void_p), ("coef_v", C.c_void_p), ("pitch", C.c_long),
                ("h", C.c_int), ("w", C.c_int), ("out_h", C.c_int), ("out_w", C.c_int), ("ksize_h", C.c_int), ("ksize_v", C.c_int),
                ("rows_max", C.c_int), ("reserved", C.c_int), ("out_off", C.c_long), ("ws_off", C.c_long)]


IMGPREP_PAD, IMGPREP_BRIGHT, IMGPREP_OUT_BF16, IMGPREP_OUT_U8, IMGPREP_TWO_PASS = 1, 2, 4, 8, 16


class ColorJitterFrame(C.Structure):
    _fields_ = [("src", C.c_void_p), ("pitch", C.c_long), ("h", C.c_int), ("w", C.c_int), ("out_off", C.c_long), ("order", C.c_int * 4),
                ("brightness", C.c_float), ("contrast", C.c_float), ("saturation", C.c_float), ("hue_shift", C.c_ubyte), ("reserved", C.c_ubyte * 3)]


COLORJITTER_LIFT = 1


class JpegmapFrame(C.Structure):
    _fields_ = [("src", C.c_void_p), ("pitch", C.c_long), ("h", C.c_int), ("w", C.c_int), ("out_off", C.c_long), ("ws_off", C.c_long)]


JPEGMAP_CV2_ORDER = 1


class LstmDesc(C.Structure):
    _fields_ = [("state_dim", C.c_int), ("hidden", C.c_int), ("layers", C.c_int), ("force_dim", C.c_int),
                ("force_pad", C.c_int), ("in_pad", C.c_int), ("cdt", C.c_int)]


_lib: Optional[C.CDLL] = None


def lib() -> C.CDLL:
    global _lib
    if _lib is not None:
        return _lib
    if not os.path.exists(LIB_PATH):
        raise VtError(f"{LIB_PATH} not found — build it with `python __graft_entry__.py` (hipcc --offload-arch=gfx950). "
                      "vlatouch has no CPU/eager fallback.")
    L = C.CDLL(LIB_PATH)
    L.vt_last_error.restype = C.c_char_p
    L.vt_version.restype = C.c_int
    for name, (res, args) in SIGNATURES.items():
        if not hasattr(L, name):
            raise VtError(f"{LIB_PATH} does not export {name} (stale build?)")
        fn = getattr(L, name)
        fn.restype = res
        fn.argtypes = args
    _lib = L
    return L


_P, _I, _L, _F, _Z = C.c_void_p, C.c_int, C.c_long, C.c_float, C.c_size_t
SIGNATURES = {
    "vt_selftest_mfma": (_I, [_P, _P]),
    "vt_prof_enable": (_I, [_I]),
    "vt_prof_collect": (_I, [_P, _P, _P, _P]),
    "vt_gemm": (_I, [_P, _P]),
    "vt_gemm_route_of": (_I, [_P]),
    "vt_gemm_route_split": (_I, [_P, _P, _P]),
    "vt_randn": (_I, [_P, _L, _P, _I, _P]),
    "vt_slice_cast": (_I, [_P, _I, _P, _I, _I, _I, _I, _I, _P]),
    "vt_cast": (_I, [_P, _I, _L, _P, _I, _L, _I, _I, _P]),
    "vt_pack_w32": (_I, [_P, _L, _P, _I, _I, _P]),
    "vt_tune": (_I, [_I, _I]),
    "vt_attention": (_I, [_P, _P]),
    "vt_attention_kvt": (_I, [_P, _P]),
    "vt_attention_kvt_part_bytes": (_Z, [_I, _I, _I, _I]),
    "vt_retile_kv": (_I, [_P, _P, _L, _P, _I, _I, _I, _P]),
    "vt_groupnorm": (_I, [_P, _P]),
    "vt_rownorm": (_I, [_P, _I, _L, _P, _I, _L, _P, _P, _I, _I, _F, _I, _P]),
    "vt_headnorm": (_I, [_P, _I, _L, _I, _L, _P, _F, _I, _P]),
    "vt_action_normalize": (_I, [_P, _P, _P, _P, _L, _I, _F, _I, _P]),
    "vt_unet_create": (_I, [_P, _P, _I, _P]),
    "vt_unet_destroy": (None, [_P]),
    "vt_unet_num_weights": (_I, [_P]),
    "vt_unet_workspace_bytes": (_Z, [_P, _I, _I]),
    "vt_unet_fused_bytes": (_Z, [_P]),
    "vt_unet_fused_pack": (_I, [_P, _P, _P]),
    "vt_unet_fused_covers": (_I, [_P, _I, _I, _I]),
    "vt_unet_fused_plan_bytes": (_Z, [_P, _I, _I, _I]),
    "vt_unet_forward": (_I, [_P, _P, _P, _F, _P, _P, _I, _I, _P, _P]),
    "vt_si_sample": (_I, [_P, _P, _P, _P, _I, _F, _I, _I, _I, _P, _I, _I, _P, _P]),
    "vt_si_sample_ex": (_I, [_P, _P, _P, _P, _I, _F, _I, _I, _I, _I, _F, _P, _I, _I, _P, _P]),
    "vt_dino_create": (_I, [_P, _P, _I, _P]),
    "vt_dino_destroy": (None, [_P]),
    "vt_dino_num_weights": (_I, [_P]),
    "vt_dino_workspace_bytes": (_Z, [_P, _I, _I]),
    "vt_dino_packed_bytes": (_Z, [_P]),
    "vt_dino_set_packed": (_I, [_P, _P, _P]),
    "vt_dino_set_range_flag": (_I, [_P, _P]),
    "vt_dino_forward": (_I, [_P, _P, _I, _I, _I, _F, _I, _I, _I, _P, _P, _P, _P, _P]),
    "vt_t5_create": (_I, [_P, _P, _I, _P]),
    "vt_t5_destroy": (None, [_P]),
    "vt_t5_num_weights": (_I, [_P]),
    "vt_t5_workspace_bytes": (_Z, [_P, _I, _I]),
    "vt_t5_forward": (_I, [_P, _P, _P, _I, _I, _P, _P, _I, _P, _P]),
    "vt_mlp": (_I, [_P, _L, _I, _I, _P, _P, _P, _I, _P, _I, _L, _I, _I, _P, _P]),
    "vt_concat_obs": (_I, [_P, _P, _I, _P, _I, _P, _I, _P, _I, _L, _I, _P]),
    "vt_lstm_create": (_I, [_P, _P, _I, _P]),
    "vt_lstm_destroy": (None, [_P]),
    "vt_lstm_num_weights": (_I, [_P]),
    "vt_lstm_workspace_bytes": (_Z, [_P, _I]),
    "vt_lstm_step": (_I, [_P, _P, _P, _P, _P, _P, _P, _I, _P, _P]),
    "vt_lstm_sequence": (_I, [_P, _P, _P, _P, _P, _P, _P, _I, _I, _P]),
    "vt_rdt_create": (_I, [_P, _P, _I, _P]),
    "vt_rdt_destroy": (None, [_P]),
    "vt_rdt_num_weights": (_I, [_P]),
    "vt_rdt_workspace_bytes": (_Z, [_P, _I, _I]),
    "vt_rdt_set_score_bounds": (_I, [_P, _P, _I]),
    "vt_rdt_set_state_precision": (_I, [_P, _I]),
    "vt_rdt_set_io_dtype": (_I, [_P, _I]),
    "vt_rdt_packed_bytes": (_Z, [_P]),
    "vt_rdt_set_packed": (_I, [_P, _P, _P]),
    "vt_rdt_set_range_flag": (_I, [_P, _P]),
    "vt_rdt_forward": (_I, [_P, _P, _P, _P, _F, _I, _P, _P, _P, _P, _I, _I, _P, _P]),
    "vt_rdt_sample": (_I, [_P, _P, _P, _P, _P, _P, _P, _P, _I, _P, _P, _I, _I, _P, _I, _I, _P, _P]),
    "vt_im2col_t": (_I, [_P, _P, _I, _I, _I, _I, _I, _I, _I, _P]),
    "vt_transpose": (_I, [_P, _P, _I, _I, _P]),
    "vt_zero_stuff": (_I, [_P, _P, _I, _I, _I, _P]),
    "vt_wflip": (_I, [_P, _P, _I, _I, _I, _P]),
    "vt_colsum": (_I, [_P, _L, _P, _I, _I, _I, _P]),
    "vt_add_": (_I, [_P, _P, _L, _P]),
    "vt_copy_cols": (_I, [_P, _L, _I, _P, _L, _I, _I, _I, _I, _P]),
    "vt_mish": (_I, [_P, _P, _P, _L, _P]),
    "vt_gn_mish_bwd": (_I, [_P, _P, _P, _P, _P, _P, _P, _P, _P, _I, _I, _I, _I, _F, _P]),
    "vt_gelu": (_I, [_P, _P, _P, _L, _P]),
    "vt_si_qsample": (_I, [_P, _P, _P, _P, _P, _P, _P, _P, _P, _I, _L, _I, _F, _P]),
    "vt_si_qsample_ex": (_I, [_P, _P, _P, _P, _P, _P, _P, _P, _P, _I, _L, _I, _F, _I, _P]),
    "vt_si_loss": (_I, [_P, _P, _P, _P, _I, _L, _P]),
    "vt_slab_sum": (_I, [_P, _I, _L, _P, _I, _P, _P]),
    "vt_adamw": (_I, [_P, _P, _P, _P, _L, _F, _F, _F, _F, _F, _I, _P]),
    "vt_ema_update": (_I, [_P, _P, _L, _F, _P]),
    "vt_train_hyper": (_I, [_F, _F, _F, _I, _F, _P]),
    "vt_adamw_dev": (_I, [_P, _P, _P, _P, _L, _P, _F, _F, _F, _F, _P]),
    "vt_adamw_ema_multi": (_I, [_P, _I, _L, _P, _F, _F, _F, _F, _P]),
    "vt_ema_update_dev": (_I, [_P, _P, _L, _P, _P]),
    "vt_posemb": (_I, [_P, _P, _I, _I, _P]),
    "vt_lstm_cell_fwd": (_I, [_P, _P, _P, _P, _P, _P, _P, _I, _I, _I, _I, _P]),
    "vt_lstm_cell_bwd": (_I, [_P, _P, _P, _P, _P, _P, _P, _I, _I, _I, _I, _P]),
    "vt_ln_bwd": (_I, [_P, _P, _P, _P, _P, _I, _I, _F, _P]),
    "vt_bcast_mid": (_I, [_P, _P, _L, _I, _I, _I, _I, _P]),
    "vt_sum_mid": (_I, [_P, _L, _I, _P, _I, _I, _I, _P]),
    "vt_mul_": (_I, [_P, _P, _L, _P]),
    "vt_mse_residual": (_I, [_P, _P, _P, _P, _P, _P, _L, _P]),
    "vt_attention_bwd": (_I, [_P, _P]),
    "vt_attention_bwd_mfma_ws_bytes": (_L, [_I, _I, _I, _I]),
    "vt_attention_bwd_mfma": (_I, [_P, _P, _L, _P]),
    "vt_rmsnorm_bwd": (_I, [_P, _P, _P, _P, _P, _I, _I, _F, _I, _I, _P]),
    "vt_headnorm_bwd": (_I, [_P, _L, _P, _L, _I, _L, _P, _P, _F, _I, _I, _P]),
    "vt_act_bwd": (_I, [_P, _P, _P, _L, _I, _I, _P]),
    "vt_ddpm_qsample": (_I, [_P, _P, _P, _P, _P, _P, _I, _P, _I, _I, _I, _I, _P]),
    "vt_timestep_embed": (_I, [_P, _P, _P, _I, _I, _I, _P]),
    "vt_add_rowvec_": (_I, [_P, _I, _P, _L, _L, _P]),
    "vt_transpose_pad": (_I, [_P, _P, _I, _I, _I, _I, _P]),
    "vt_colsum_dt": (_I, [_P, _I, _L, _P, _I, _I, _P]),
    "vt_add_dt": (_I, [_P, _P, _L, _I, _P]),
    "vt_gemm_tn_plan": (_I, [_I, _I, _I, _P]),
    "vt_gemm_tn": (_I, [_P, _L, _P, _L, _I, _I, _I, _I, _P, _P, _P, _L, _P]),
    "vt_copy_cols_dt": (_I, [_P, _L, _L, _P, _L, _L, _L, _L, _I, _P]),
    "vt_grad_clip_multi": (_I, [_P, _I, _L, _F, _P, _P, _P]),
    "vt_mse_loss": (_I, [_P, _P, _P, _P, _L, _I, _P]),
    "vt_mse_loss_scaled": (_I, [_P, _P, _P, _P, _L, _I, _F, _P]),
    "vt_grad_unscale_clip_multi": (_I, [_P, _I, _L, _F, _F, _P, _P, _P, _P]),
    "vt_grad_accum_multi": (_I, [_P, _P, _I, _L, _F, _I, _P]),
    "vt_ema_multi": (_I, [_P, _I, _L, _P, _P]),
    "vt_grad_fold_pack_multi": (_I, [_P, _P, _I, _L, _F, _I, _P, _P]),
    "vt_grad_unpack_multi": (_I, [_P, _P, _I, _L, _P]),
    "vt_adamw8_ema_multi": (_I, [_P, _P, _P, _I, _L, _P, _F, _F, _F, _F, _P]),
    "vt_adam8_quantize": (_I, [_P, _P, _P, _P, _I, _L, _P]),
    "vt_adam8_dequantize": (_I, [_P, _P, _P, _I, _P, _L, _P]),
    "vt_sample_metrics": (_I, [_P, _I, _P, _P, _P, _P, _I, _I, _I, _I, _P, _P, _P, _P, _P, _P]),
    "vt_imgprep_workspace_bytes": (_Z, [_P, _I, _I, _I]),
    "vt_imgprep": (_I, [_P, _P, _I, _I, _P, C.c_uint, _I, _P, _P, _Z, _P]),
    "vt_colorjitter_workspace_bytes": (_Z, [_I]),
    "vt_colorjitter": (_I, [_P, _P, _I, _I, _P, _P, _Z, _P]),
    "vt_jpegmap_workspace_bytes": (_Z, [_P, _I]),
    "vt_jpegmap": (_I, [_P, _P, _I, _I, _I, _P, _P, _Z, _P]),
    "vt_rdt_batch": (_I, [_P, _P, _P, _P, _P, _P, _P, _I, _I, _I, _I, _I, _I, _I, C.c_double, _P, _I, _P, _P, _P, _P, _P, _P, _P, _P]),
    "vt_ctrl_batch": (_I, [_P, _P, _P, _P, _P, _P, _I, C.c_longlong, _I, _I, _I, C.c_longlong, _P, _F, _I, _I, _I, _I, _P, _I, _P, _I, _P, _P, _P, _P,
                           _P, _P]),
    "vt_ctrl_pixsum": (_I, [_P, C.c_longlong, _I, _P, _P]),
    "vt_marker_workspace_bytes": (_Z, [_I, _I, _I, _I]),
    "vt_marker_detect": (_I, [_P, _I, _I, _I, _I, _I, C.c_double, C.c_double, _I, _P, _P, _I, _P, _P, _P]),
    "vt_marker_displacement": (_I, [_P, _P, _I, _I, _P, _I, _P, _P, _P]),
}


class RdtDesc(C.Structure):
    _fields_ = [("hidden", C.c_int), ("depth", C.c_int), ("heads", C.c_int), ("horizon", C.c_int), ("out_dim", C.c_int),
                ("state_dim", C.c_int), ("lang_dim", C.c_int), ("img_dim", C.c_int), ("max_lang_len", C.c_int), ("img_len", C.c_int),
                ("n_lang", C.c_int), ("n_img", C.c_int), ("n_state", C.c_int), ("cdt", C.c_int), ("adt", C.c_int), ("rms_mode", C.c_int)]


def check(code: int, what: str = "") -> None:
    if code != 0:
        raise VtError(f"{what or 'vlatouch'} failed with code {code}: {lib().vt_last_error().decode()}")


def stream_ptr(device=None) -> C.c_void_p:
    return C.c_void_p(torch.cuda.current_stream(device).cuda_stream)


def ptr(t: Optional[torch.Tensor]) -> C.c_void_p:
    return C.c_void_p(0 if t is None else t.data_ptr())


def dt_code(dtype: torch.dtype) -> int:
    if dtype == torch.float32:
        return F32
    if dtype == torch.bfloat16:
        return BF16
    if dtype == torch.float16:
        return F16
    raise VtError(f"unsupported dtype {dtype}")


def torch_dtype(code: int) -> torch.dtype:
    return {F32: torch.float32, F32X3: torch.float32, BF16: torch.bfloat16, F16: torch.float16}[code]


def ptr_array(tensors: Sequence[Optional[torch.Tensor]]):
    arr = (C.c_void_p * len(tensors))()
    for i, t in enumerate(tensors):
        arr[i] = 0 if t is None else t.data_ptr()
    return arr


def require_gpu(device) -> torch.device:
    device = torch.device(device)
    if device.type != "cuda" or not torch.cuda.is_available():
        raise VtError("vlatouch runs only on an AMD GPU through libvlatouch_hip.so (device must be 'cuda'; "
                      "no CPU fallback exists)")
    lib()
    return device
```

### vla-touch_amd/vlatouch/ops.py

```python
from __future__ import annotations

import ctypes as C
from typing import Optional

import torch

from . import _lib as L


def _es(t: torch.Tensor) -> int:
    return t.element_size()


def gemm(a: torch.Tensor, w: torch.Tensor, bias: Optional[torch.Tensor] = None, *, act: int = L.ACT_NONE,
         colscale: Optional[torch.Tensor] = None, residual: Optional[torch.Tensor] = None,
         out: Optional[torch.Tensor] = None, out_dtype: Optional[torch.dtype] = None, splitk: int = 1,
         headnorm=None, cmap=None, wp: Optional[torch.Tensor] = None, sk_ws: Optional[torch.Tensor] = None,
         sk_cnt: Optional[torch.Tensor] = None, xn=None, rs=None) -> torch.Tensor:
    assert a.dim() == 2 and w.dim() == 2 and a.shape[1] == w.shape[1]
    M, K = a.shape
    N = w.shape[0]
    out_dtype = out_dtype or (torch.float32 if splitk > 1 else a.dtype)
    if out is None:
        out = torch.empty((splitk, M, N) if splitk > 1 else (M, N), dtype=out_dtype, device=a.device)
    p = L.GemmParams()
    p.A, p.W, p.C = a.data_ptr(), w.data_ptr(), out.data_ptr()
    p.M, p.N, p.K = M, N, K
    p.lda, p.ldw, p.ldc = a.stride(0), w.stride(0), N
    p.bias = 0 if bias is None else bias.data_ptr()
    p.colscale = 0 if colscale is None else colscale.data_ptr()
    if residual is not None:
        assert residual.dtype == out_dtype
        p.residual, p.ldr = residual.data_ptr(), residual.stride(0)
    p.act, p.groups, p.splitk = act, 1, splitk
    p.c_slab = M * N
    p.a_dtype, p.w_dtype, p.c_dtype = L.dt_code(a.dtype), L.dt_code(w.dtype), L.dt_code(out_dtype)
    if headnorm is not None:
        w0, c0, w1, c1, eps, mode = headnorm
        p.hn_w0, p.hn_c0_end = w0.data_ptr(), c0
        p.hn_w1, p.hn_c1_end = (0 if w1 is None else w1.data_ptr()), c1
        p.hn_eps, p.hn_mode = eps, mode
    if cmap is not None:
        p.cmap, p.cmap_T = cmap
    if wp is not None:
        assert wp.numel() == w.numel() and wp.dtype == w.dtype
        p.Wp = wp.data_ptr()
    if sk_ws is not None and sk_cnt is not None:
        assert sk_cnt.dtype == torch.int32
        p.sk_ws, p.sk_ws_bytes, p.sk_cnt, p.sk_cnt_n = sk_ws.data_ptr(), sk_ws.numel() * sk_ws.element_size(), sk_cnt.data_ptr(), sk_cnt.numel()
    if xn is not None:
        xo, gain, part = xn[:3]
        p.rs_mode = xn[3] if len(xn) > 3 else L.NORM_RMS_MEANSQ
        assert xo.shape == (M, N) and xo.dtype == a.dtype and gain.dtype == torch.float32 and part.dtype == torch.float32 and part.shape == (M, 2 * N // 128, 2) and part.is_contiguous()
        p.xn_out, p.xn_ld, p.xn_gain, p.xn_part = xo.data_ptr(), xo.stride(0), gain.data_ptr(), part.data_ptr()
    if rs is not None:
        part, eps = rs[0], rs[1]
        assert part.dtype == torch.float32 and part.shape[0] == M and part.dim() == 3 and part.shape[2] == 2 and part.is_contiguous()
        p.rs_part, p.rs_n, p.rs_inv_k, p.rs_eps = part.data_ptr(), part.shape[1], 1.0 / K, eps
        p.rs_mode = rs[2] if len(rs) > 2 else L.NORM_RMS_MEANSQ
    L.check(L.lib().vt_gemm(C.byref(p), L.stream_ptr(a.device)), "vt_gemm")
    return out


def _grouped(t: torch.Tensor, grouped: bool, what: str):
    assert t.dim() == (3 if grouped else 2) and t.stride(-1) == 1, f"{what}: expected a {'3' if grouped else '2'}-D view with unit inner stride"
    return t.data_ptr(), (t.stride(0) if grouped else 0), t.stride(-2)


def gemm_block_params(a: torch.Tensor, w: torch.Tensor, out: torch.Tensor, bias: Optional[torch.Tensor] = None, *, w_code: Optional[int] = None,
                      act: int = L.ACT_NONE, colscale: Optional[torch.Tensor] = None, residual: Optional[torch.Tensor] = None, splitk: int = 1,
                      conv: Optional[dict] = None) -> L.GemmParams:
    grouped = out.dim() - (1 if splitk > 1 else 0) == 3
    p = L.GemmParams()
    p.W, p.w_gs, p.ldw = _grouped(w, grouped, "w")
    if conv is None:
        p.A, p.a_gs, p.lda = _grouped(a, grouped, "a")
        M, K = a.shape[-2:]
    else:
        taps, cin, tout = conv["taps"], conv["cin"], conv["tout"]
        assert a.dim() == (4 if grouped else 3) and a.shape[-1] == cin and a.stride(-1) == 1 and a.stride(-3) == a.shape[-2] * a.stride(-2)
        p.A, p.a_gs, p.lda = a.data_ptr(), (a.stride(0) if grouped else 0), a.stride(-2)
        M, K = a.shape[-3] * tout, taps * cin
        p.taps, p.cin, p.tout, p.tin = taps, cin, tout, a.shape[-2]
        p.stride, p.off0, p.tstep = conv.get("stride", 1), conv.get("off0", 0), conv.get("tstep", 1)
    N = w.shape[-2]
    assert w.shape[-1] == K and tuple(out.shape[-2:]) == (M, N)
    G = out.shape[-3] if grouped else 1
    assert not grouped or (a.shape[0] == G and w.shape[0] == G)
    p.M, p.N, p.K = M, N, K
    if splitk > 1:
        assert out.shape[0] == splitk and out.dtype == torch.float32
        p.c_slab = out.stride(0)
        p.C, p.c_gs, p.ldc = _grouped(out[0], grouped, "out")
    else:
        p.C, p.c_gs, p.ldc = _grouped(out, grouped, "out")
        p.c_slab = M * N
    if bias is not None:
        assert bias.dtype == torch.float32 and bias.dim() == (2 if grouped else 1) and bias.shape[-1] == N and bias.stride(-1) == 1
        p.bias, p.bias_gs = bias.data_ptr(), (bias.stride(0) if grouped else 0)
    if colscale is not None:
        assert colscale.dtype == torch.float32 and colscale.shape == (N,) and colscale.stride(0) == 1
        p.colscale = colscale.data_ptr()
    if residual is not None:
        assert residual.dtype == out.dtype and residual.shape == (out[0].shape if splitk > 1 else out.shape)
        p.residual, p.r_gs, p.ldr = _grouped(residual, grouped, "residual")
    p.act, p.groups, p.splitk = act, G, splitk
    p.a_dtype, p.w_dtype, p.c_dtype = L.dt_code(a.dtype), (L.dt_code(w.dtype) if w_code is None else w_code), L.dt_code(out.dtype)
    return p


def gemm_route(p: L.GemmParams) -> str:
    return L.ROUTE_NAMES[L.lib().vt_gemm_route_of(C.addressof(p))]


def gemm_block(a: torch.Tensor, w: torch.Tensor, out: torch.Tensor, bias: Optional[torch.Tensor] = None, *, route: Optional[str] = None, **fields) -> str:
    p = gemm_block_params(a, w, out, bias, **fields)
    got = gemm_route(p)
    assert route is None or got == route, f"the dispatcher sends this block to {got}, the caller expects {route}"
    L.check(L.lib().vt_gemm(C.byref(p), L.stream_ptr(out.device)), "vt_gemm")
    return got


def groupnorm_block_params(slabs: torch.Tensor, bias: Optional[torch.Tensor], gamma: torch.Tensor, beta: torch.Tensor, out: torch.Tensor, *, B: int, T: int,
                           ngroups: int = 8, film: Optional[torch.Tensor] = None, film_off: int = 0, residual: Optional[torch.Tensor] = None,
                           eps: float = 1e-5) -> L.GnParams:
    S, nets, M, Cc = slabs.shape
    assert M == B * T and slabs.dtype == torch.float32 and slabs.stride(3) == 1 and out.shape == (nets, M, Cc) and out.stride(2) == 1
    vecs = [v for v in (bias, gamma, beta) if v is not None]
    assert all(v.dtype == torch.float32 and v.shape == (nets, Cc) and v.stride(1) == 1 and v.stride(0) == gamma.stride(0) for v in vecs)
    p = L.GnParams()
    p.P, p.nslabs, p.slab_stride, p.p_gs, p.ldp = slabs.data_ptr(), S, slabs.stride(0), slabs.stride(1), slabs.stride(2)
    p.bias = 0 if bias is None else bias.data_ptr()
    p.gamma, p.beta, p.vec_gs = gamma.data_ptr(), beta.data_ptr(), gamma.stride(0)
    if film is not None:
        assert film.dtype == torch.float32 and film.dim() == 3 and film.shape[:2] == (nets, B) and film.stride(2) == 1 and 0 <= film_off <= film.shape[2] - 2 * Cc
        p.film, p.film_gs, p.film_ld, p.film_off = film.data_ptr(), film.stride(0), film.stride(1), film_off
    if residual is not None:
        assert residual.dtype == out.dtype and residual.shape == out.shape and residual.stride(2) == 1
        p.residual, p.r_gs, p.ldr = residual.data_ptr(), residual.stride(0), residual.stride(1)
    p.out, p.o_gs, p.ldo, p.out_dtype = out.data_ptr(), out.stride(0), out.stride(1), L.dt_code(out.dtype)
    p.B, p.T, p.C, p.ngroups, p.nets, p.eps = B, T, Cc, ngroups, nets, eps
    return p


def groupnorm_block(slabs: torch.Tensor, bias, gamma, beta, out: torch.Tensor, **fields) -> None:
    p = groupnorm_block_params(slabs, bias, gamma, beta, out, **fields)
    L.check(L.lib().vt_groupnorm(C.byref(p), L.stream_ptr(out.device)), "vt_groupnorm")


class DeviceRng:

    def __init__(self, seed: int, device="cuda"):
        self.device = L.require_gpu(device)
        self.state = torch.tensor([seed & 0x7FFFFFFFFFFFFFFF, 0], dtype=torch.int64, device=self.device)

    def normal_(self, out: torch.Tensor, round_bf16: bool = False) -> torch.Tensor:
        assert out.dtype == torch.float32 and out.is_contiguous() and out.device.type == "cuda"
        L.check(L.lib().vt_randn(L.ptr(out), out.numel(), L.ptr(self.state), int(round_bf16), L.stream_ptr(out.device)), "vt_randn")
        return out


def slice_cast(x: torch.Tensor, T: int, D: int, out: Optional[torch.Tensor] = None) -> torch.Tensor:
    assert x.dim() == 3 and x.is_contiguous()
    B, Tin, Din = x.shape
    if out is None:
        out = torch.empty(B, T, D, dtype=torch.float32, device=x.device)
    L.check(L.lib().vt_slice_cast(L.ptr(x), L.dt_code(x.dtype), L.ptr(out), B, Tin, Din, T, D, L.stream_ptr(x.device)), "vt_slice_cast")
    return out


def cast(x: torch.Tensor, dtype: torch.dtype, out: Optional[torch.Tensor] = None) -> torch.Tensor:
    assert x.is_contiguous()
    if out is None:
        out = torch.empty(x.shape, dtype=dtype, device=x.device)
    cols = x.shape[-1]
    rows = x.numel() // cols
    L.check(L.lib().vt_cast(L.ptr(x), L.dt_code(x.dtype), cols, L.ptr(out), L.dt_code(dtype), cols, rows, cols, L.stream_ptr(x.device)), "vt_cast")
    return out


def pack_w32(w: torch.Tensor) -> torch.Tensor:
    assert w.dim() == 2 and w.stride(1) == 1 and w.element_size() == 2
    out = torch.empty(w.numel(), dtype=w.dtype, device=w.device)
    L.check(L.lib().vt_pack_w32(L.ptr(w), w.stride(0), L.ptr(out), w.shape[0], w.shape[1], L.stream_ptr(w.device)), "vt_pack_w32")
    return out


def conv1d_cl(x: torch.Tensor, w_packed: torch.Tensor, bias: Optional[torch.Tensor], *, taps: int, cin: int, tout: int,
              stride: int = 1, off0: int = 0, tstep: int = 1, out_dtype: Optional[torch.dtype] = None, splitk: int = 1) -> torch.Tensor:
    B, tin, c = x.shape
    assert c == cin and x.is_contiguous()
    N = w_packed.shape[0]
    out_dtype = out_dtype or (torch.float32 if splitk > 1 else x.dtype)
    out = torch.empty((splitk, B, tout, N) if splitk > 1 else (B, tout, N), dtype=out_dtype, device=x.device)
    p = L.GemmParams()
    p.A, p.W, p.C = x.data_ptr(), w_packed.data_ptr(), out.data_ptr()
    p.M, p.N, p.K = B * tout, N, taps * cin
    p.lda, p.ldw, p.ldc = cin, taps * cin, N
    p.taps, p.cin, p.tout, p.tin, p.stride, p.off0, p.tstep = taps, cin, tout, tin, stride, off0, tstep
    p.bias = 0 if bias is None else bias.data_ptr()
    p.groups, p.splitk = 1, splitk
    p.c_slab = B * tout * N
    p.a_dtype, p.w_dtype, p.c_dtype = L.dt_code(x.dtype), L.dt_code(w_packed.dtype), L.dt_code(out_dtype)
    L.check(L.lib().vt_gemm(C.byref(p), L.stream_ptr(x.device)), "vt_gemm(conv)")
    return out


def attention(q: torch.Tensor, k: torch.Tensor, v: torch.Tensor, *, scale: Optional[float] = None,
              kmask: Optional[torch.Tensor] = None) -> torch.Tensor:
    B, Nq, H, hd = q.shape
    Nk = k.shape[1]
    assert hd in (64, 80, 96) and q.stride(3) == 1 and k.stride(3) == 1 and v.stride(3) == 1
    o = torch.empty(B, Nq, H * hd, dtype=q.dtype, device=q.device)
    p = L.AttnParams()
    p.Q, p.K, p.V, p.O = q.data_ptr(), k.data_ptr(), v.data_ptr(), o.data_ptr()
    p.q_bs, p.q_rs, p.q_hs = q.stride(0), q.stride(1), q.stride(2)
    p.k_bs, p.k_rs, p.k_hs = k.stride(0), k.stride(1), k.stride(2)
    p.v_bs, p.v_rs, p.v_hs = v.stride(0), v.stride(1), v.stride(2)
    p.o_bs, p.o_rs = Nq * H * hd, H * hd
    p.hd = hd
    km = None
    if kmask is not None:
        km = kmask.to(torch.uint8).contiguous()
        p.kmask, p.km_bs = km.data_ptr(), Nk
    p.B, p.H, p.Nq, p.Nk = B, H, Nq, Nk
    p.scale = scale if scale is not None else hd ** -0.5
    p.dtype = L.dt_code(q.dtype)
    L.check(L.lib().vt_attention(C.byref(p), L.stream_ptr(q.device)), "vt_attention")
    return o


def rownorm(x: torch.Tensor, w: torch.Tensor, b: Optional[torch.Tensor], eps: float, mode: int = L.NORM_LAYER,
            out_dtype: Optional[torch.dtype] = None) -> torch.Tensor:
    assert x.dim() == 2 and x.stride(1) == 1
    out_dtype = out_dtype or x.dtype
    y = torch.empty(x.shape, dtype=out_dtype, device=x.device)
    L.check(L.lib().vt_rownorm(L.ptr(x), L.dt_code(x.dtype), x.stride(0), L.ptr(y), L.dt_code(out_dtype), y.stride(0), L.ptr(w), L.ptr(b),
                               x.shape[0], x.shape[1], eps, mode, L.stream_ptr(x.device)), "vt_rownorm")
    return y


def headnorm_(x: torch.Tensor, heads: int, w: torch.Tensor, eps: float = 1e-6, mode: int = L.NORM_RMS_MEANSQ, tok_stride: Optional[int] = None,
              tokens: Optional[int] = None) -> None:
    tok_stride = tok_stride if tok_stride is not None else x.stride(-2)
    tokens = tokens if tokens is not None else x.numel() // x.shape[-1]
    L.check(L.lib().vt_headnorm(L.ptr(x), L.dt_code(x.dtype), tok_stride, heads, tokens, L.ptr(w), eps, mode, L.stream_ptr(x.device)), "vt_headnorm")


def groupnorm_cl(slabs: torch.Tensor, bias, gamma, beta, *, B: int, T: int, ngroups: int = 8, film: Optional[torch.Tensor] = None,
                 residual: Optional[torch.Tensor] = None, out_dtype: torch.dtype = torch.float32, eps: float = 1e-5) -> torch.Tensor:
    S, M, Cc = slabs.shape
    assert M == B * T
    out = torch.empty(M, Cc, dtype=out_dtype, device=slabs.device)
    p = L.GnParams()
    p.P, p.nslabs, p.slab_stride, p.p_gs, p.ldp = slabs.data_ptr(), S, M * Cc, 0, Cc
    p.bias = 0 if bias is None else bias.data_ptr()
    p.gamma, p.beta, p.vec_gs = gamma.data_ptr(), beta.data_ptr(), 0
    if film is not None:
        p.film, p.film_ld, p.film_off, p.film_gs = film.data_ptr(), film.stride(0), 0, 0
    if residual is not None:
        assert residual.dtype == out_dtype
        p.residual, p.ldr, p.r_gs = residual.data_ptr(), residual.stride(0), 0
    p.out, p.ldo, p.o_gs, p.out_dtype = out.data_ptr(), Cc, 0, L.dt_code(out_dtype)
    p.B, p.T, p.C, p.ngroups, p.nets, p.eps = B, T, Cc, ngroups, 1, eps
    L.check(L.lib().vt_groupnorm(C.byref(p), L.stream_ptr(slabs.device)), "vt_groupnorm")
    return out


def mfma_selftest(device="cuda"):
    err = torch.full((2,), -1.0, dtype=torch.float32, device=device)
    L.check(L.lib().vt_selftest_mfma(L.ptr(err), L.stream_ptr(err.device)), "vt_selftest_mfma")
    return err.cpu().tolist()
```

Measured before the change: 407.7.

## Add wide-N PW GEMM kernel computing three column tiles per block

Adds a new GEMM kernel variant for the PW route in which each 256-thread block computes three adjacent BN column tiles against one A tile. The A tile is staged once in a six-slot LDS ring while the weights use a three-deep register ring, and the epilogue writes the three output tiles one after another through a shared LDS tile. It is on by default for 16-bit outputs when the tile count is between 100 and 256. The aim is to cut repeated A loads and the number of blocks on mid-sized GEMMs. The cost is higher register pressure, a smaller grid, and vmcnt bookkeeping that must stay correct.

```diff
diff --git a/include/vlatouch.h b/include/vlatouch.h
--- a/include/vlatouch.h
+++ b/include/vlatouch.h
@@ -34,6 +34,7 @@
        VT_ROUTE_ROWSPLIT = 10 };
 int vt_gemm_route_of(const void* params);
 int vt_gemm_route_split(const void* params, int* head_route, int* tail_route);
+int vt_gemm_pw_wide_of(const void* params);
 int vt_pack_w32(const void* W, long ldw, void* out, int N, int K, vt_stream_t stream);
 int vt_tune(int knob, int value);
 
diff --git a/vla-touch_amd/csrc/vt_api.hip b/vla-touch_amd/csrc/vt_api.hip
--- a/vla-touch_amd/csrc/vt_api.hip
+++ b/vla-touch_amd/csrc/vt_api.hip
@@ -24,6 +24,11 @@
   if (!params) return VT_ROUTE_BAD_ARG;
   return vt_gemm_route(*reinterpret_cast<const VtGemmParams*>(params));
 }
+int vt_gemm_pw_wide_of(const void* params) {
+  if (!params) return 0;
+  const VtGemmParams& p = *reinterpret_cast<const VtGemmParams*>(params);
+  return vt_gemm_route(p) == VT_GEMM_PW && vt_gemm_pw_takes_wide(p);
+}
 int vt_gemm_route_split(const void* params, int* head_route, int* tail_route) {
   if (!params || !head_route || !tail_route) return vt_fail(VT_ERR_ARG, "vt_gemm_route_split: null argument");
   const VtGemmParams& p = *reinterpret_cast<const VtGemmParams*>(params);
@@ -34,7 +39,8 @@
   return VT_OK;
 }
 int vt_tune(int knob, int value) {
-  if (knob == 1 && (value == 0 || value == 4 || value == 8)) { vt_gemm_pw_tune(value); return VT_OK; }
+  if (knob == 1 && (value == 0 || value == 4 || value == 8)) { vt_gemm_pw_tune(1, value); return VT_OK; }
+  if (knob == 10) { vt_gemm_pw_tune(10, value); return VT_OK; }
   if (knob == 2 || knob == 8) { vt_gemm_route_tune(knob, value); return VT_OK; }
   if (knob == 4) { vt_gemm_pws_tune(value); return VT_OK; }
   if (knob == 6) { vt_attn_kvt_tune(value); return VT_OK; }
diff --git a/vla-touch_amd/csrc/vt_common.h b/vla-touch_amd/csrc/vt_common.h
--- a/vla-touch_amd/csrc/vt_common.h
+++ b/vla-touch_amd/csrc/vt_common.h
@@ -101,6 +101,10 @@
   asm volatile("s_waitcnt vmcnt(%[n])" : "+v"(w[0]), "+v"(w[1]), "+v"(w[2]), "+v"(w[3]), "+v"(w[4]), "+v"(w[5]), "+v"(w[6]), "+v"(w[7]) : [n] "i"(VT_VMCNT(N)) : "memory");
 }
 
+template <int N> __device__ __forceinline__ void vt_wait_vm(int4_t (&w)[12]) {
+  asm volatile("s_waitcnt vmcnt(%[n])" : "+v"(w[0]), "+v"(w[1]), "+v"(w[2]), "+v"(w[3]), "+v"(w[4]), "+v"(w[5]), "+v"(w[6]), "+v"(w[7]), "+v"(w[8]), "+v"(w[9]), "+v"(w[10]), "+v"(w[11]) : [n] "i"(VT_VMCNT(N)) : "memory");
+}
+
 template <int OFF, bool FIRST>
 __device__ __forceinline__ void wload(int4_t& d, const unsigned voff, const char* sbase) {
   if constexpr (FIRST) asm volatile("s_nop 4\n\tglobal_load_dwordx4 %0, %1, %2 offset:%3" : "=v"(d) : "v"(voff), "s"(sbase), "i"(OFF) : "memory");
diff --git a/vla-touch_amd/csrc/vt_gemm_pw.hip b/vla-touch_amd/csrc/vt_gemm_pw.hip
--- a/vla-touch_amd/csrc/vt_gemm_pw.hip
+++ b/vla-touch_amd/csrc/vt_gemm_pw.hip
@@ -13,6 +13,120 @@
 constexpr int A_TILE = BM * 128;
 constexpr int OPS = BM / 8 / 4 + 4;
 
+__device__ __forceinline__ void pw_tile_of(const int total_tiles, const int tiles_n, const int tiles_per_group, const int GM, int& grp, int& tm, int& tn) {
+  int bid = blockIdx.x;
+  if ((total_tiles & 7) == 0) bid = (bid & 7) * (total_tiles >> 3) + (bid >> 3);
+  grp = bid / tiles_per_group;
+  const int t_in = bid - grp * tiles_per_group;
+  const int tiles_m = tiles_per_group / tiles_n;
+  const int sr = t_in / (GM * tiles_n);
+  const int gmr = min(GM, tiles_m - sr * GM);
+  const int r_in = t_in - sr * GM * tiles_n;
+  tn = r_in / gmr;
+  tm = sr * GM + (r_in - tn * gmr);
+}
+__device__ __forceinline__ void pw_asrc(int (&asrc)[5], const VtGemmParams& p, const int m0, const int wave, const int lane) {
+#pragma unroll
+  for (int e = 0; e < 5; ++e) {
+    const int r = (wave + 4 * e) * 8 + (lane >> 3);
+    const int c = (lane & 7) ^ ((r >> 1) & 7);
+    asrc[e] = (int)(((long)(min(m0 + r, p.M - 1) - m0) * p.lda + c * 8) * 2);
+  }
+}
+__device__ __forceinline__ void pw_issue_a(const __amdgpu_buffer_rsrc_t rsA, char* smem, const int b, const int wave, const int (&asrc)[5], const int kt) {
+#pragma unroll
+  for (int e = 0; e < 5; ++e)
+    __builtin_amdgcn_raw_ptr_buffer_load_lds(rsA, (lds_void*)(smem + b * A_TILE + (wave + 4 * e) * 1024), 16, asrc[e], kt * (BK * 2), 0, 0);
+}
+__device__ __forceinline__ void pw_foff(int (&foff)[4], const int l31, const int hk) {
+  const int xr = (l31 >> 1) & 7;
+#pragma unroll
+  for (int s = 0; s < 4; ++s) foff[s] = l31 * 128 + (((s * 2 + hk) ^ xr) * 16);
+}
+__device__ __forceinline__ void pw_frags(int4_t (&f)[TMW], const char* smem, const int b, const int off) {
+#pragma unroll
+  for (int j = 0; j < TMW; ++j) f[j] = *reinterpret_cast<const int4_t*>(smem + b * A_TILE + j * 4096 + off);
+}
+constexpr int PW_RSV = (BM * 16 + 255) / 256;
+__device__ __forceinline__ void pw_rs_request(float4 (&rsv)[PW_RSV], const VtGemmParams& p, const int m0, const int tid) {
+  const int h2 = p.rs_n >> 1, nq = BM * h2;
+#pragma unroll
+  for (int i = 0; i < PW_RSV; ++i) {
+    const int q = tid + 256 * i;
+    const int row = q / h2, c = q - row * h2;
+    rsv[i] = q < nq ? *reinterpret_cast<const float4*>(p.rs_part + ((long)min(m0 + row, p.M - 1) * p.rs_n + 2 * c) * 2) : make_float4(0.f, 0.f, 0.f, 0.f);
+  }
+}
+__device__ __forceinline__ void pw_rstd(float (&rs)[TMW], const float4 (&rsv)[PW_RSV], float* tile, const VtGemmParams& p, const int tid, const int l31) {
+  float2* pair = reinterpret_cast<float2*>(tile + BM);
+  const int h2 = p.rs_n >> 1;
+#pragma unroll
+  for (int i = 0; i < PW_RSV; ++i) {
+    const int q = tid + 256 * i;
+    if (q < BM * h2) {
+      const float dS = rsv[i].y - rsv[i].w;
+      pair[q] = make_float2(rsv[i].x + rsv[i].z + (p.rs_mode == 2 ? dS * dS * (1.0f / 128.0f) : 0.f), rsv[i].y + rsv[i].w);
+    }
+  }
+  __syncthreads();
+  if (tid < BM) {
+    float var;
+    if (p.rs_mode == 2) {
+      float na = 0.f, mean = 0.f, m2 = 0.f;
+      for (int c = 0; c < h2; ++c) {
+        const float2 v = pair[tid * h2 + c];
+        const float delta = v.y * (1.0f / 128.0f) - mean, nt = na + 128.0f;
+        mean += delta * (128.0f / nt);
+        m2 += v.x + delta * delta * (na * 128.0f / nt);
+        na = nt;
+      }
+      var = m2 / (1.0f / p.rs_inv_k - 1.0f);
+    } else {
+      float sq = 0.f;
+      for (int c = 0; c < h2; ++c) sq += pair[tid * h2 + c].x;
+      var = sq * p.rs_inv_k;
+    }
+    tile[tid] = rsqrtf(var + p.rs_eps);
+  }
+  __syncthreads();
+#pragma unroll
+  for (int j = 0; j < TMW; ++j) rs[j] = tile[j * 32 + l31];
+  __syncthreads();
+}
+template <bool SCALE>
+__device__ __forceinline__ void pw_tile_put(float* tile, const float16_t (&acc)[TMW], const float (&rs)[TMW], const int wave, const int l31, const int hk) {
+#pragma unroll
+  for (int j = 0; j < TMW; ++j) {
+    const int m = j * 32 + l31;
+    const float r = SCALE ? rs[j] : 1.f;
+#pragma unroll
+    for (int rq = 0; rq < 4; ++rq) {
+      const int n4 = wave * 8 + rq * 2 + hk;
+      *reinterpret_cast<float4*>(tile + m * BN + ((n4 ^ (m & 7)) * 4)) =
+          make_float4(acc[j][rq * 4] * r, acc[j][rq * 4 + 1] * r, acc[j][rq * 4 + 2] * r, acc[j][rq * 4 + 3] * r);
+    }
+  }
+}
+template <typename TC, bool ACT>
+__device__ __forceinline__ void pw_tile_rows(const VtGemmParams& p, const float* tile, const int half, const int c4, const int rbase, const float4 b4, const float4 cs4,
+                                             const float* hw, const float4 hw4, TC* Cg, const TC* Rg, const int m0, const int n, const int ncol0, const bool col_ok) {
+  if constexpr (ACT) {
+#pragma unroll 2
+    for (int it = 0; it < BM / 8; ++it) {
+      const int row = rbase + it * 4;
+      const float4 x = *reinterpret_cast<const float4*>(tile + row * BN + (((half * 16 + c4) ^ (row & 7)) * 4));
+      vt_epi_segment<TC, 0, true>(p, x, b4, cs4, hw, hw4, Cg, Rg, m0 + row, n, ncol0, col_ok);
+    }
+  } else {
+#pragma unroll 4
+    for (int it = 0; it < BM / 8; ++it) {
+      const int row = rbase + it * 4;
+      const float4 x = *reinterpret_cast<const float4*>(tile + row * BN + (((half * 16 + c4) ^ (row & 7)) * 4));
+      vt_epi_segment<TC, 0, false>(p, x, b4, cs4, hw, hw4, Cg, Rg, m0 + row, n, ncol0, col_ok);
+    }
+  }
+}
+
 template <typename T16, typename TC, int NB, int FUSE = 0>
 __global__ __launch_bounds__(256, 1) void gemm_pw_kernel(const VtGemmParams p, const int tiles_n, const int tiles_per_group, const int total_tiles, const int GM) {
   constexpr int SMEM = NB * A_TILE > BM * BN * 4 ? NB * A_TILE : BM * BN * 4;
@@ -21,15 +135,8 @@
   const int wave = __builtin_amdgcn_readfirstlane(tid >> 6);
   const int l31 = lane & 31, hk = lane >> 5;
 
-  int bid = blockIdx.x;
-  if ((total_tiles & 7) == 0) bid = (bid & 7) * (total_tiles >> 3) + (bid >> 3);
-  const int grp = bid / tiles_per_group;
-  const int t_in = bid - grp * tiles_per_group;
-  const int tiles_m = tiles_per_group / tiles_n;
-  const int sr = t_in / (GM * tiles_n);
-  const int gmr = min(GM, tiles_m - sr * GM);
-  const int r_in = t_in - sr * GM * tiles_n;
-  const int tn = r_in / gmr, tm = sr * GM + (r_in - tn * gmr);
+  int grp, tm, tn;
+  pw_tile_of(total_tiles, tiles_n, tiles_per_group, GM, grp, tm, tn);
   const int m0 = tm * BM, n0 = tn * BN;
 
   const uint16_t* A = reinterpret_cast<const uint16_t*>(p.A) + (long)grp * p.a_gs;
@@ -37,12 +144,7 @@
 
   const __amdgpu_buffer_rsrc_t rsA = __builtin_amdgcn_make_buffer_rsrc((void*)(A + (long)m0 * p.lda), 0, 0x7fffffff, 0x00020000);
   int asrc[5];
-#pragma unroll
-  for (int e = 0; e < 5; ++e) {
-    const int r = (wave + 4 * e) * 8 + (lane >> 3);
-    const int c = (lane & 7) ^ ((r >> 1) & 7);
-    asrc[e] = (int)(((long)(min(m0 + r, p.M - 1) - m0) * p.lda + c * 8) * 2);
-  }
+  pw_asrc(asrc, p, m0, wave, lane);
   const char* wbase = reinterpret_cast<const char*>(p.Wp) + ((long)grp * p.w_gs) * 2 + ((long)(n0 / 32 + wave) * (p.K / 16)) * 1024;
   wbase = VT_UNIFORM_PTR(wbase);
   const unsigned wvoff = lane * 16;
@@ -50,9 +152,7 @@
   int4_t wb[NB][4];
   auto issue = [&](const int kt, auto bc) {
     constexpr int b = decltype(bc)::value;
-#pragma unroll
-    for (int e = 0; e < 5; ++e)
-      __builtin_amdgcn_raw_ptr_buffer_load_lds(rsA, (lds_void*)(smem + b * A_TILE + (wave + 4 * e) * 1024), 16, asrc[e], kt * (BK * 2), 0, 0);
+    pw_issue_a(rsA, smem, b, wave, asrc, kt);
     const char* sb = wbase + (long)kt * 4096;
     wload<0, true>(wb[b][0], wvoff, sb);
     wload<1024, false>(wb[b][1], wvoff, sb);
@@ -60,14 +160,9 @@
     wload<3072, false>(wb[b][3], wvoff, sb);
   };
 
-  const int xr = (l31 >> 1) & 7;
   int foff[4];
-#pragma unroll
-  for (int s = 0; s < 4; ++s) foff[s] = l31 * 128 + (((s * 2 + hk) ^ xr) * 16);
-  auto frags = [&](int4_t (&f)[TMW], const int b, const int s) {
-#pragma unroll
-    for (int j = 0; j < TMW; ++j) f[j] = *reinterpret_cast<const int4_t*>(smem + b * A_TILE + j * 4096 + foff[s]);
-  };
+  pw_foff(foff, l31, hk);
+  auto frags = [&](int4_t (&f)[TMW], const int b, const int s) { pw_frags(f, smem, b, foff[s]); };
 
   float16_t acc[TMW];
 #pragma unroll
@@ -84,20 +179,13 @@
   int4_t af[2][TMW];
   frags(af[0], 0, 0);
 
-  constexpr int RSV = FUSE == 2 ? (BM * 16 + 255) / 256 : 1;
-  float4 rsv[RSV];
+  float4 rsv[PW_RSV];
   auto sub = [&](const int t, auto uc, auto tailc) {
     constexpr int U = decltype(uc)::value;
     constexpr bool TAIL = decltype(tailc)::value;
     if constexpr (!TAIL || U == 0) issue(t + NB - 1, std::integral_constant<int, (U + NB - 1) % NB>{});
     if constexpr (FUSE == 2 && TAIL && U == NB - 2) {
-      const int h2 = p.rs_n >> 1, nq = BM * h2;
-#pragma unroll
-      for (int i = 0; i < RSV; ++i) {
-        const int q = tid + 256 * i;
-        const int row = q / h2, c = q - row * h2;
-        rsv[i] = q < nq ? *reinterpret_cast<const float4*>(p.rs_part + ((long)min(m0 + row, p.M - 1) * p.rs_n + 2 * c) * 2) : make_float4(0.f, 0.f, 0.f, 0.f);
-      }
+      pw_rs_request(rsv, p, m0, tid);
     }
 #pragma unroll
     for (int s = 0; s < 4; ++s) {
@@ -125,42 +213,7 @@
   float rs[TMW];
 #pragma unroll
   for (int j = 0; j < TMW; ++j) rs[j] = 1.f;
-  if constexpr (FUSE == 2) {
-    float2* pair = reinterpret_cast<float2*>(tile + BM);
-    const int h2 = p.rs_n >> 1;
-#pragma unroll
-    for (int i = 0; i < RSV; ++i) {
-      const int q = tid + 256 * i;
-      if (q < BM * h2) {
-        const float dS = rsv[i].y - rsv[i].w;
-        pair[q] = make_float2(rsv[i].x + rsv[i].z + (p.rs_mode == 2 ? dS * dS * (1.0f / 128.0f) : 0.f), rsv[i].y + rsv[i].w);
-      }
-    }
-    __syncthreads();
-    if (tid < BM) {
-      float var;
-      if (p.rs_mode == 2) {
-        float na = 0.f, mean = 0.f, m2 = 0.f;
-        for (int c = 0; c < h2; ++c) {
-          const float2 v = pair[tid * h2 + c];
-          const float delta = v.y * (1.0f / 128.0f) - mean, nt = na + 128.0f;
-          mean += delta * (128.0f / nt);
-          m2 += v.x + delta * delta * (na * 128.0f / nt);
-          na = nt;
-        }
-        var = m2 / (1.0f / p.rs_inv_k - 1.0f);
-      } else {
-        float sq = 0.f;
-        for (int c = 0; c < h2; ++c) sq += pair[tid * h2 + c].x;
-        var = sq * p.rs_inv_k;
-      }
-      tile[tid] = rsqrtf(var + p.rs_eps);
-    }
-    __syncthreads();
-#pragma unroll
-    for (int j = 0; j < TMW; ++j) rs[j] = tile[j * 32 + l31];
-    __syncthreads();
-  }
+  if constexpr (FUSE == 2) pw_rstd(rs, rsv, tile, p, tid, l31);
   const int half = wave & 1, c4 = lane & 15;
   const int ncol0 = n0 + half * 64, n = ncol0 + c4 * 4;
   const bool col_ok = n < p.N;
@@ -205,25 +258,10 @@
       if ((unsigned)i * 16384u < share) pfv[i] = __builtin_amdgcn_raw_buffer_load_b32(rsP, (i * 256 + tid) * 64, 0, 0);
   }
   __builtin_amdgcn_sched_barrier(0);
-#pragma unroll
-  for (int j = 0; j < TMW; ++j) {
-    const int m = j * 32 + l31;
-    const float r = FUSE == 2 ? rs[j] : 1.f;
-#pragma unroll
-    for (int rq = 0; rq < 4; ++rq) {
-      const int n4 = wave * 8 + rq * 2 + hk;
-      *reinterpret_cast<float4*>(tile + m * BN + ((n4 ^ (m & 7)) * 4)) =
-          make_float4(acc[j][rq * 4] * r, acc[j][rq * 4 + 1] * r, acc[j][rq * 4 + 2] * r, acc[j][rq * 4 + 3] * r);
-    }
-  }
+  pw_tile_put<FUSE == 2>(tile, acc, rs, wave, l31, hk);
   __syncthreads();
   if (p.act != VT_ACT_NONE) {
-#pragma unroll 2
-    for (int it = 0; it < BM / 8; ++it) {
-      const int row = rbase + it * 4;
-      const float4 x = *reinterpret_cast<const float4*>(tile + row * BN + (((half * 16 + c4) ^ (row & 7)) * 4));
-      vt_epi_segment<TC, 0, true>(p, x, b4, cs4, hw, hw4, Cg, Rg, m0 + row, n, ncol0, col_ok);
-    }
+    pw_tile_rows<TC, true>(p, tile, half, c4, rbase, b4, cs4, hw, hw4, Cg, Rg, m0, n, ncol0, col_ok);
   } else if (FUSE == 1 && PRE && use_pre) {
     if constexpr (PRE && FUSE == 1) {
       T16* Xn = reinterpret_cast<T16*>(p.xn_out);
@@ -265,15 +303,154 @@
       vt_epi_segment<TC, 0, false>(p, x, b4, cs4, hw, hw4, Cg, nullptr, m0 + row, n, ncol0, col_ok, &rpre[PRE ? it : 0]);
     }
   } else {
-#pragma unroll 4
-    for (int it = 0; it < BM / 8; ++it) {
-      const int row = rbase + it * 4;
-      const float4 x = *reinterpret_cast<const float4*>(tile + row * BN + (((half * 16 + c4) ^ (row & 7)) * 4));
-      vt_epi_segment<TC, 0, false>(p, x, b4, cs4, hw, hw4, Cg, Rg, m0 + row, n, ncol0, col_ok);
-    }
+    pw_tile_rows<TC, false>(p, tile, half, c4, rbase, b4, cs4, hw, hw4, Cg, Rg, m0, n, ncol0, col_ok);
   }
 #pragma unroll
   for (int i = 0; i < PFN; ++i) asm volatile("" :: "v"(pfv[i]));
+}
+
+constexpr int WG = 3;
+constexpr int OPSW = BM / 8 / 4 + 4 * WG;
+
+constexpr int NBW = 3, NBA = 6;
+
+template <typename T16, int FUSE, int R>
+__global__ __launch_bounds__(256, 1) void gemm_pw_wide_kernel(const VtGemmParams p, const int tiles_n, const int total_tiles, const int GM) {
+  static_assert(FUSE == 0 || FUSE == 2, "plain, or the consumer of an RMSNorm hand-off");
+  static_assert(R == 4 || R == 6 || R == 8, "the k-tiles behind the last whole turn of the A ring");
+  static_assert(NBA % NBW == 0 && NBA > NBW, "tile t: A slot t % NBA, weight buffer t % NBW, one turn of the A ring per unrolled loop body");
+  static_assert(2 * OPSW + 4 * WG < 64, "vmcnt is a 6-bit counter");
+  static_assert(NBA * A_TILE >= BM * BN * 4, "the epilogue's tile lies inside the ring");
+  __shared__ __attribute__((aligned(16))) char smem[NBA * A_TILE];
+  const int tid = threadIdx.x, lane = tid & 63;
+  const int wave = __builtin_amdgcn_readfirstlane(tid >> 6);
+  const int l31 = lane & 31, hk = lane >> 5;
+
+  int grp, tm, tn;
+  pw_tile_of(total_tiles, tiles_n, total_tiles, GM, grp, tm, tn);
+  const int m0 = tm * BM, n0 = tn * (WG * BN);
+  const uint16_t* A = reinterpret_cast<const uint16_t*>(p.A);
+  const int nk = p.K / BK;
+
+  const __amdgpu_buffer_rsrc_t rsA = __builtin_amdgcn_make_buffer_rsrc((void*)(A + (long)m0 * p.lda), 0, 0x7fffffff, 0x00020000);
+  int asrc[5];
+  pw_asrc(asrc, p, m0, wave, lane);
+  const char* wbase[WG];
+  static_for<WG>([&](auto gc) {
+    const char* w = reinterpret_cast<const char*>(p.Wp) + ((long)(n0 / 32 + 4 * decltype(gc)::value + wave) * (p.K / 16)) * 1024;
+    wbase[decltype(gc)::value] = VT_UNIFORM_PTR(w);
+  });
+  const unsigned wvoff = lane * 16;
+
+  int4_t wb[NBW][4 * WG];
+  auto wissue = [&](const int kt, auto bc, auto sc) __attribute__((always_inline)) {
+    constexpr int b = decltype(bc)::value, s = decltype(sc)::value;
+    static_for<WG>([&](auto gc) {
+      constexpr int g = decltype(gc)::value;
+      wload<s * 1024, true>(wb[b][4 * g + s], wvoff, wbase[g] + (long)kt * 4096);
+    });
+  };
+
+  int foff[4];
+  pw_foff(foff, l31, hk);
+  float16_t acc[WG][TMW];
+#pragma unroll
+  for (int g = 0; g < WG; ++g)
+#pragma unroll
+    for (int j = 0; j < TMW; ++j)
+#pragma unroll
+      for (int r = 0; r < 16; ++r) acc[g][j][r] = 0.f;
+
+  static_for<NBW>([&](auto bc) {
+    pw_issue_a(rsA, smem, decltype(bc)::value, wave, asrc, decltype(bc)::value);
+    static_for<4>([&](auto sc) { wissue(decltype(bc)::value, bc, sc); });
+  });
+  vt_wait_vm<OPSW>(wb[0]);
+  vt_wait_vm<OPSW>(wb[1]);
+  __builtin_amdgcn_sched_barrier(0);
+  __builtin_amdgcn_s_barrier();
+  __builtin_amdgcn_sched_barrier(0);
+  int4_t fr[3];
+  auto fread = [&](const int slot, const int f, int4_t& d) __attribute__((always_inline)) {
+    d = *reinterpret_cast<const int4_t*>(smem + slot * A_TILE + (f % TMW) * 4096 + foff[f / TMW]);
+  };
+  fread(0, 0, fr[0]);
+  fread(0, 1, fr[1]);
+
+  auto sub = [&](const int t, auto sac, auto leftc) __attribute__((always_inline)) {
+    constexpr int SA = decltype(sac)::value, U = SA % NBW, LEFT = decltype(leftc)::value;
+    constexpr bool more = LEFT >= 3;
+    if constexpr (more) pw_issue_a(rsA, smem, (SA + 3) % NBA, wave, asrc, t + 3);
+    static_for<4>([&](auto sc) {
+      constexpr int s = decltype(sc)::value;
+      static_for<TMW>([&](auto jc) {
+        constexpr int j = decltype(jc)::value, f = TMW * s + j, F = 20 * SA + f;
+        if constexpr (f + 2 < 4 * TMW) fread(SA, f + 2, fr[(F + 2) % 3]);
+        else if constexpr (LEFT >= 1) fread((SA + 1) % NBA, f + 2 - 4 * TMW, fr[(F + 2) % 3]);
+#pragma unroll
+        for (int g = 0; g < WG; ++g) acc[g][j] = mma32<T16>(wb[U][4 * g + s], fr[F % 3], acc[g][j]);
+      });
+#pragma unroll
+      for (int i = 0; i < TMW; ++i) {
+        __builtin_amdgcn_sched_group_barrier(0x100, 1, 0);
+        __builtin_amdgcn_sched_group_barrier(0x008, WG, 0);
+      }
+      __builtin_amdgcn_sched_barrier(0);
+      if constexpr (more) wissue(t + 3, std::integral_constant<int, U>{}, sc);
+      __builtin_amdgcn_sched_barrier(0);
+    });
+    if constexpr (more) vt_wait_vm<2 * 4 * WG + BM / 8 / 4>(wb[(U + 1) % NBW]);
+    else if constexpr (LEFT == 2) vt_wait_vm<4 * WG>(wb[(U + 1) % NBW]);
+    else if constexpr (LEFT == 1) vt_wait_vm<0>(wb[(U + 1) % NBW]);
+    __builtin_amdgcn_sched_barrier(0);
+    __builtin_amdgcn_s_barrier();
+    __builtin_amdgcn_sched_barrier(0);
+  };
+  int t = 0;
+  for (; t + NBA + 2 < nk; t += NBA) static_for<NBA>([&](auto uc) { sub(t + decltype(uc)::value, uc, std::integral_constant<int, 3>{}); });
+  static_for<R>([&](auto uc) {
+    constexpr int U = decltype(uc)::value;
+    sub(t + U, std::integral_constant<int, U % NBA>{}, std::integral_constant<int, R - 1 - U>{});
+  });
+
+  int tid_e = threadIdx.x;
+  asm volatile("" : "+v"(tid_e));
+  const int lane_e = tid_e & 63, l31_e = lane_e & 31, hk_e = lane_e >> 5;
+  float* tile = reinterpret_cast<float*>(smem);
+  float rs[TMW];
+#pragma unroll
+  for (int j = 0; j < TMW; ++j) rs[j] = 1.f;
+  if constexpr (FUSE == 2) {
+    float4 rsv[PW_RSV];
+    pw_rs_request(rsv, p, m0, tid_e);
+    pw_rstd(rs, rsv, tile, p, tid_e, l31_e);
+  }
+  const int half = wave & 1, c4 = lane_e & 15;
+  const int rbase = (wave >> 1) * (BM / 2) + (lane_e >> 4);
+  T16* Cg = reinterpret_cast<T16*>(p.C);
+  const T16* Rg = reinterpret_cast<const T16*>(p.residual);
+  const float4 zero4 = make_float4(0.f, 0.f, 0.f, 0.f), one4 = make_float4(1.f, 1.f, 1.f, 1.f);
+  const float* hw[WG];
+  float4 b4[WG], cs4[WG], hw4[WG];
+#pragma unroll
+  for (int g = 0; g < WG; ++g) {
+    const int ncol0 = n0 + g * BN + half * 64, n = ncol0 + c4 * 4;
+    hw[g] = nullptr;
+    if (p.hn_w0 && ncol0 < p.hn_c0_end) hw[g] = p.hn_w0;
+    else if (p.hn_w1 && ncol0 >= p.hn_c0_end && ncol0 < p.hn_c1_end) hw[g] = p.hn_w1;
+    b4[g] = p.bias ? *reinterpret_cast<const float4*>(p.bias + n) : zero4;
+    cs4[g] = p.colscale ? *reinterpret_cast<const float4*>(p.colscale + n) : one4;
+    hw4[g] = hw[g] ? *reinterpret_cast<const float4*>(hw[g] + c4 * 4) : one4;
+  }
+  static_for<WG>([&](auto gc) {
+    constexpr int g = decltype(gc)::value;
+    const int ncol0 = n0 + g * BN + half * 64, n = ncol0 + c4 * 4;
+    if constexpr (g > 0) __syncthreads();
+    pw_tile_put<FUSE == 2>(tile, acc[g], rs, wave, l31_e, hk_e);
+    __syncthreads();
+    if (p.act != VT_ACT_NONE) pw_tile_rows<T16, true>(p, tile, half, c4, rbase, b4[g], cs4[g], hw[g], hw4[g], Cg, Rg, m0, n, ncol0, true);
+    else pw_tile_rows<T16, false>(p, tile, half, c4, rbase, b4[g], cs4[g], hw[g], hw4[g], Cg, Rg, m0, n, ncol0, true);
+  });
 }
 
 __global__ void pack_w32_kernel(const uint16_t* __restrict__ W, const long ldw, uint16_t* __restrict__ out, const int N, const int K) {
@@ -291,8 +468,12 @@
 }
 
 static int g_vt_pw_nb = 0;
-
-void vt_gemm_pw_tune(int ring) { g_vt_pw_nb = ring; }
+static int g_vt_pw_wide = 1;
+
+void vt_gemm_pw_tune(int knob, int value) {
+  if (knob == 1) g_vt_pw_nb = value;
+  else g_vt_pw_wide = value != 0;
+}
 
 bool vt_gemm_pw_fits(const VtGemmParams& p) {
   if (!p.Wp || p.cmap || p.groups != 1) return false;
@@ -302,12 +483,36 @@
   return tiles >= 100 && tiles * 8 >= rounds * 256 * 7;
 }
 
+bool vt_gemm_pw_wide_fits(const VtGemmParams& p) {
+  if (!p.Wp || p.cmap || p.groups != 1 || p.c_dtype == VT_F32 || p.xn_out) return false;
+  if (p.N % (WG * BN) || p.K % (8 * BK) || p.lda >= (1 << 21)) return false;
+  const long tiles = (long)((p.M + BM - 1) / BM) * (p.N / (WG * BN));
+  return tiles >= 100 && tiles <= 256;
+}
+
+bool vt_gemm_pw_takes_wide(const VtGemmParams& p) { return g_vt_pw_wide && vt_gemm_pw_wide_fits(p); }
+
 int vt_gemm_pw_launch(const VtGemmParams& p, hipStream_t s) {
   const int tiles_n = p.N / BN, tiles_m = (p.M + BM - 1) / BM;
   const int per_group = tiles_n * tiles_m, total = per_group * p.groups;
   const int gm = 4;
   VtProfScope prof(3, p, s);
   const bool c16 = p.c_dtype != VT_F32;
+  if (vt_gemm_pw_takes_wide(p)) {
+    const int wn = p.N / (WG * BN);
+    const dim3 g(tiles_m * wn), b(256);
+    int left = p.K / BK;
+    while (left > NBA + 2) left -= NBA;
+#define VT_PWW_R(T16, F) do { if (left == 4) hipLaunchKernelGGL((gemm_pw_wide_kernel<T16, F, 4>), g, b, 0, s, p, wn, tiles_m * wn, gm); \
+                              else if (left == 6) hipLaunchKernelGGL((gemm_pw_wide_kernel<T16, F, 6>), g, b, 0, s, p, wn, tiles_m * wn, gm); \
+                              else hipLaunchKernelGGL((gemm_pw_wide_kernel<T16, F, 8>), g, b, 0, s, p, wn, tiles_m * wn, gm); } while (0)
+#define VT_PWW_GO(T16) do { if (p.rs_part) VT_PWW_R(T16, 2); else VT_PWW_R(T16, 0); } while (0)
+    DISPATCH_T16(p.a_dtype, T16,
+                 VT_PWW_GO(T16));
+#undef VT_PWW_GO
+#undef VT_PWW_R
+    return vt_check_launch();
+  }
 #define VT_PW_GO(T16, TC) do { if (g_vt_pw_nb == 8) hipLaunchKernelGGL((gemm_pw_kernel<T16, TC, 8>), dim3(total), dim3(256), 0, s, p, tiles_n, per_group, total, gm); \
                                else hipLaunchKernelGGL((gemm_pw_kernel<T16, TC, 4>), dim3(total), dim3(256), 0, s, p, tiles_n, per_group, total, gm); } while (0)
   if (p.xn_out || p.rs_part) {
diff --git a/vla-touch_amd/csrc/vt_gemm_route.h b/vla-touch_amd/csrc/vt_gemm_route.h
--- a/vla-touch_amd/csrc/vt_gemm_route.h
+++ b/vla-touch_amd/csrc/vt_gemm_route.h
@@ -27,6 +27,7 @@
 bool vt_gemm_pt_one_round(const VtGemmParams& p);
 bool vt_gemm_ppk_fits(const VtGemmParams& p);
 bool vt_gemm_pw_fits(const VtGemmParams& p);
+bool vt_gemm_pw_wide_fits(const VtGemmParams& p);
 bool vt_gemm_pws_fits(const VtGemmParams& p);
 bool vt_gemm_f32r_fits(const VtGemmParams& p);
 
@@ -38,5 +39,6 @@
 int vt_gemm_ppk_launch(const VtGemmParams& p, hipStream_t s);
 int vt_gemm_pw_launch(const VtGemmParams& p, hipStream_t s);
 int vt_gemm_pws_launch(const VtGemmParams& p, hipStream_t s);
-void vt_gemm_pw_tune(int ring);
+bool vt_gemm_pw_takes_wide(const VtGemmParams& p);
+void vt_gemm_pw_tune(int knob, int value);
 void vt_gemm_pws_tune(int split);
diff --git a/vla-touch_amd/csrc/vt_gemm_route.hip b/vla-touch_amd/csrc/vt_gemm_route.hip
--- a/vla-touch_amd/csrc/vt_gemm_route.hip
+++ b/vla-touch_amd/csrc/vt_gemm_route.hip
@@ -40,7 +40,7 @@
   if (p.pf_ptr && p.pf_bytes >= (1ul << 31)) return VT_GEMM_BAD_ARG;
   const bool hn = p.hn_w0 || p.hn_w1;
   const bool lds = vt_gemm_lds_fits(p);
-  const bool pw = lds && g_pw_on && vt_gemm_pw_fits(p);
+  const bool pw = lds && g_pw_on && (vt_gemm_pw_fits(p) || vt_gemm_pw_wide_fits(p));
   if (p.xn_out || p.rs_part) {
     if (p.groups != 1 || (p.xn_out && (!p.xn_gain || !p.xn_part || p.c_dtype != VT_F32 || !p.residual || p.act != VT_ACT_NONE || hn || p.xn_ld % 4)) ||
         (p.rs_part && (p.rs_n < 4 || p.rs_n > 32 || p.rs_n % 4)) || !pw)
diff --git a/vla-touch_amd/vlatouch/_lib.py b/vla-touch_amd/vlatouch/_lib.py
--- a/vla-touch_amd/vlatouch/_lib.py
+++ b/vla-touch_amd/vlatouch/_lib.py
@@ -192,6 +192,7 @@
     "vt_prof_collect": (_I, [_P, _P, _P, _P]),
     "vt_gemm": (_I, [_P, _P]),
     "vt_gemm_route_of": (_I, [_P]),
+    "vt_gemm_pw_wide_of": (_I, [_P]),
     "vt_gemm_route_split": (_I, [_P, _P, _P]),
     "vt_randn": (_I, [_P, _L, _P, _I, _P]),
     "vt_slice_cast": (_I, [_P, _I, _P, _I, _I, _I, _I, _I, _P]),
diff --git a/vla-touch_amd/vlatouch/ops.py b/vla-touch_amd/vlatouch/ops.py
--- a/vla-touch_amd/vlatouch/ops.py
+++ b/vla-touch_amd/vlatouch/ops.py
@@ -69,7 +69,7 @@
 
 def gemm_block_params(a: torch.Tensor, w: torch.Tensor, out: torch.Tensor, bias: Optional[torch.Tensor] = None, *, w_code: Optional[int] = None,
                       act: int = L.ACT_NONE, colscale: Optional[torch.Tensor] = None, residual: Optional[torch.Tensor] = None, splitk: int = 1,
-                      conv: Optional[dict] = None) -> L.GemmParams:
+                      conv: Optional[dict] = None, wp: Optional[torch.Tensor] = None, headnorm=None, rs=None) -> L.GemmParams:
     grouped = out.dim() - (1 if splitk > 1 else 0) == 3
     p = L.GemmParams()
     p.W, p.w_gs, p.ldw = _grouped(w, grouped, "w")
@@ -106,11 +106,28 @@
         p.residual, p.r_gs, p.ldr = _grouped(residual, grouped, "residual")
     p.act, p.groups, p.splitk = act, G, splitk
     p.a_dtype, p.w_dtype, p.c_dtype = L.dt_code(a.dtype), (L.dt_code(w.dtype) if w_code is None else w_code), L.dt_code(out.dtype)
+    if wp is not None:
+        assert not grouped and wp.numel() == w.numel() and wp.dtype == w.dtype and w.is_contiguous()
+        p.Wp = wp.data_ptr()
+    if headnorm is not None:
+        w0, c0, w1, c1, eps, mode = headnorm
+        p.hn_w0, p.hn_c0_end = w0.data_ptr(), c0
+        p.hn_w1, p.hn_c1_end = (0 if w1 is None else w1.data_ptr()), c1
+        p.hn_eps, p.hn_mode = eps, mode
+    if rs is not None:
+        part, eps = rs[0], rs[1]
+        assert part.dtype == torch.float32 and part.shape[0] == M and part.dim() == 3 and part.shape[2] == 2 and part.is_contiguous()
+        p.rs_part, p.rs_n, p.rs_inv_k, p.rs_eps = part.data_ptr(), part.shape[1], 1.0 / K, eps
+        p.rs_mode = rs[2] if len(rs) > 2 else L.NORM_RMS_MEANSQ
     return p
 
 
 def gemm_route(p: L.GemmParams) -> str:
     return L.ROUTE_NAMES[L.lib().vt_gemm_route_of(C.addressof(p))]
+
+
+def gemm_pw_wide(p: L.GemmParams) -> bool:
+    return bool(L.lib().vt_gemm_pw_wide_of(C.addressof(p)))
 
 
 def gemm_block(a: torch.Tensor, w: torch.Tensor, out: torch.Tensor, bias: Optional[torch.Tensor] = None, *, route: Optional[str] = None, **fields) -> str:
```

New measurement: 408.7, median of 2. About the same (+0.3%).
